# juanmc2005/diart

Hardware: NVIDIA H100
Metric: audio-seconds/sec (real-time factor) at 5s/0.5s step, batch 256 (higher is better)
Workload: dtype f32

## Files before the change

### diart_b200/_lib.py

```python
from __future__ import annotations

import ctypes as C
import os
from typing import Dict, Optional

import numpy as np
import torch

_HERE = os.path.dirname(os.path.abspath(__file__))
LIB_PATH = os.path.join(_HERE, "libdiartb200.so")

_lib: Optional[C.CDLL] = None


class DgTensor(C.Structure):
    _fields_ = [("name", C.c_char_p), ("data", C.c_void_p), ("numel", C.c_int64)]


_P = C.c_void_p
SIGNATURES = {
    "dg_last_error": (C.c_char_p, []),
    "dg_version": (C.c_int, []),
    "dg_launch_count": (C.c_int64, []),
    "dg_profile_enable": (C.c_int, [C.c_int]),
    "dg_profile_report": (C.c_int, [C.c_char_p, C.c_int]),
    "dg_selftest_gemm_tc": (C.c_int, [C.c_int, C.c_int, C.c_int, C.c_int, C.c_int, C.c_int, C.POINTER(C.c_float),
                                      C.POINTER(C.c_float)]),
    "dg_selftest_gemm_tc_grid": (C.c_int, [C.c_int, C.c_int, C.c_int, C.c_int, C.c_int, C.c_int, C.POINTER(C.c_int)]),
    "dg_selftest_gemm_tc_bounds": (C.c_int, [C.c_int, C.c_int, C.c_int, C.c_int, C.POINTER(C.c_int), C.POINTER(C.c_int),
                                             C.POINTER(C.c_int)]),
    "dg_selftest_wgmma_row_shift": (C.c_int, [C.c_int, C.POINTER(C.c_uint)]),
    "dg_selftest_wgmma_b_row_shift": (C.c_int, [C.c_int, C.POINTER(C.c_uint)]),
    "dg_selftest_gemm_tc_pool3_simt": (C.c_int, [C.c_int, C.c_int, C.c_int, C.c_int, C.c_int, C.POINTER(C.c_float),
                                                 C.POINTER(C.c_float), C.POINTER(C.c_int)]),
    "dg_selftest_gemm_tc_halo": (C.c_int, [C.c_int, C.c_int, C.c_int, C.c_int, C.c_int, C.c_int, C.POINTER(C.c_int),
                                           C.POINTER(C.c_int)]),
    "dg_selftest_split_f16_host": (C.c_int, [_P, C.c_longlong, _P, _P]),
    "dg_seg_create": (C.c_int, [C.POINTER(DgTensor), C.c_int, C.c_int, C.POINTER(_P)]),
    "dg_seg_dims": (C.c_int, [_P, C.c_int, C.POINTER(C.c_int), C.POINTER(C.c_int)]),
    "dg_seg_set_powerset": (C.c_int, [_P, C.c_int, C.c_int]),
    "dg_seg_forward": (C.c_int, [_P, _P, C.c_int, C.c_int, _P, _P]),
    "dg_seg_destroy": (C.c_int, [_P]),
    "dg_emb_create": (C.c_int, [C.POINTER(DgTensor), C.c_int, C.c_int, C.c_int, C.POINTER(_P)]),
    "dg_emb_dims": (C.c_int, [_P, C.c_int, C.POINTER(C.c_int), C.POINTER(C.c_int)]),
    "dg_emb_forward": (C.c_int, [_P, _P, _P, C.c_int, C.c_int, C.c_int, C.c_int, C.c_int, C.c_float, _P, _P]),
    "dg_emb_forward_rows": (C.c_int, [_P, _P, _P, C.c_int, C.c_int, C.c_int, _P, _P]),
    "dg_emb_destroy": (C.c_int, [_P]),
    "dg_emb_debug_trunk": (C.c_int, [_P, _P, C.c_int, C.c_int, C.c_int, _P, C.c_int64, _P]),
    "dg_seg_debug_stage": (C.c_int, [_P, _P, C.c_int, C.c_int, C.c_int, C.c_int, _P, C.c_int64, _P]),
    "dg_emb_debug_stage": (C.c_int, [_P, _P, _P, C.c_int, C.c_int, C.c_int, C.c_int, C.c_int, C.c_int, _P, C.c_int64, _P]),
    "dg_selftest_sinc_filters_host": (C.c_int, [_P, _P, _P]),
    "dg_selftest_fbank_tables_host": (C.c_int, [_P, _P]),
    "dg_osp": (C.c_int, [_P, C.c_int, C.c_int, C.c_int, C.c_float, C.c_float, C.c_int, _P, _P]),
    "dg_normalize_embeddings": (C.c_int, [_P, C.c_int, C.c_int, C.c_float, _P, _P]),
    "dg_cluster_create": (C.c_int, [C.c_int, C.c_int, C.c_double, C.c_double, C.c_double, C.c_int, C.POINTER(_P)]),
    "dg_cluster_set_metric": (C.c_int, [_P, C.c_int]),
    "dg_cluster_step": (C.c_int, [_P, _P, _P, C.c_int, C.c_int, C.c_int, _P, _P, _P]),
    "dg_cluster_reset": (C.c_int, [_P]),
    "dg_cluster_get_state": (C.c_int, [_P, _P, _P, C.POINTER(C.c_int)]),
    "dg_cluster_set_state": (C.c_int, [_P, _P, _P, C.c_int]),
    "dg_cluster_destroy": (C.c_int, [_P]),
    "dg_cluster_record_len": (C.c_int, [_P]),
    "dg_cluster_export_delta": (C.c_int, [_P, _P, _P]),
    "dg_cluster_merge": (C.c_int, [_P, _P, C.c_int, C.c_int, _P, C.c_int, _P]),
    "dg_pipeline_identity_export": (C.c_int, [_P, _P, _P]),
    "dg_pipeline_identity_merge": (C.c_int, [_P, _P, C.c_int, C.c_int, _P]),
    "dg_pipeline_create": (C.c_int, [_P, _P, _P, C.c_float, C.c_float, C.c_int, C.POINTER(_P)]),
    "dg_pipeline_set_hop": (C.c_int, [_P, C.c_int]),
    "dg_pipeline_step": (C.c_int, [_P, _P, C.c_int, C.c_int, _P, _P, _P, _P, _P]),
    "dg_pipeline_step_host": (C.c_int, [_P, _P, C.c_int, C.c_int, _P, _P, _P, _P]),
    "dg_pipeline_submit": (C.c_int, [_P, _P, C.c_int, C.c_int, _P]),
    "dg_pipeline_collect": (C.c_int, [_P, C.POINTER(_P), C.POINTER(_P), C.POINTER(_P), _P]),
    "dg_pipeline_collect_copy": (C.c_int, [_P, _P, _P, _P, _P]),
    "dg_pipeline_submit_host": (C.c_int, [_P, _P, C.c_int, C.c_int]),
    "dg_pipeline_collect_host": (C.c_int, [_P, _P, _P, _P]),
    "dg_pipeline_destroy": (C.c_int, [_P]),
    "dg_pipeline_nets_sets": (C.c_int, [_P, _P, C.c_int, C.c_int, C.c_int, _P, _P, _P, _P, C.c_int64, _P]),
    "dg_post_create": (C.c_int, [C.c_int, C.c_int, C.c_int, C.c_int, _P, C.c_double, C.c_int, C.POINTER(_P)]),
    "dg_post_step": (C.c_int, [_P, _P, _P, C.c_int, _P, _P, _P, C.c_int, C.POINTER(C.c_int), _P]),
    "dg_post_reset": (C.c_int, [_P]),
    "dg_post_destroy": (C.c_int, [_P]),
    "dg_stream_create": (C.c_int, [C.c_int, C.c_int, C.c_int, C.c_int, C.POINTER(_P)]),
    "dg_stream_push_host": (C.c_int, [_P, _P, C.c_int]),
    "dg_stream_available": (C.c_int, [_P]),
    "dg_stream_windows": (C.c_int, [_P, C.c_int, _P, _P]),
    "dg_stream_reset": (C.c_int, [_P]),
    "dg_stream_destroy": (C.c_int, [_P]),
    "dg_pipeline_submit_stream": (C.c_int, [_P, _P, C.c_int]),
    "dg_pipeline_call_stream": (C.c_int, [_P, _P, _P, C.c_int, _P, _P, _P, C.c_int, C.POINTER(C.c_int), _P, _P]),
    "dg_pipeline_call_host": (C.c_int, [_P, _P, _P, C.c_int, C.c_int, _P, _P, _P, C.c_int, C.POINTER(C.c_int), _P, _P]),
    "dg_pipeline_last_call_h2d_bytes": (C.c_int64, [_P]),
    "dg_resample_create": (C.c_int, [C.c_int, C.c_int, _P, C.c_int, C.c_int, C.POINTER(_P)]),
    "dg_resample_out_len": (C.c_int64, [_P, C.c_int64]),
    "dg_resample_forward": (C.c_int, [_P, _P, C.c_int, C.c_int64, _P, _P]),
    "dg_resample_destroy": (C.c_int, [_P]),
    "dg_stream_create_resampled": (C.c_int, [C.c_int, C.c_int, _P, C.c_int, C.c_int, C.POINTER(_P)]),
    "dg_stream_crop_host": (C.c_int, [_P, C.c_int, _P, _P]),
    "dg_sweep_create": (C.c_int, [C.c_int, C.c_int, C.c_int, C.c_int, C.c_int, _P, C.c_int, C.POINTER(_P)]),
    "dg_sweep_run": (C.c_int, [_P, _P, _P, C.c_int, _P, C.c_int, _P, _P, _P, _P, _P, C.c_int, C.POINTER(C.c_int), _P]),
    "dg_sweep_destroy": (C.c_int, [_P]),
    "dg_sweep_set_scored_regions": (C.c_int, [_P, C.c_int, _P, _P]),
    "dg_sweep_set_trial_sets": (C.c_int, [_P, C.c_int, _P, C.c_int]),
    "dg_sweep_set_seeds": (C.c_int, [_P, C.c_int, _P, _P]),
    "dg_sweep_set_identities": (C.c_int, [_P, C.c_int, _P]),
    "dg_sweep_score": (C.c_int, [_P, _P, _P, C.c_int, _P, C.c_int, _P, _P, _P, C.c_double, C.c_double, _P, _P, C.c_int,
                                 C.c_int, _P, _P, _P, C.c_int, _P]),
    "dg_sweep_run_files": (C.c_int, [_P, _P, _P, C.c_int, C.c_int, _P, _P, C.c_int, _P, _P, _P, _P, _P, C.c_int,
                                     C.POINTER(C.c_int), _P]),
    "dg_sweep_score_files": (C.c_int, [_P, _P, _P, C.c_int, C.c_int, _P, _P, C.c_int, _P, _P, _P, _P, C.c_double, _P, _P,
                                       _P, _P, _P, _P, _P, C.c_int, _P]),
    "dg_sweep_state_order": (C.c_int, [C.c_int, _P, C.c_int, _P]),
    "dg_sweep_run_latencies": (C.c_int, [_P, _P, _P, C.c_int, C.c_int, _P, C.c_int, C.c_int, _P, _P, _P, C.c_int, _P, _P,
                                         _P, _P, C.c_int, C.POINTER(C.c_int), _P]),
    "dg_sweep_score_latencies": (C.c_int, [_P, _P, _P, C.c_int, C.c_int, _P, C.c_int, C.c_int, _P, _P, _P, C.c_int, _P, _P,
                                           _P, _P, C.c_double, _P, _P, _P, _P, _P, _P]),
    "dg_sweep_check_latencies": (C.c_int, [C.c_int, C.c_int, _P, C.c_int, C.c_int, _P, _P, _P, C.c_int, C.c_int]),
    "dg_vad_sweep_curve_latencies": (C.c_int, [_P, _P, C.c_int, C.c_int, _P, C.c_int, C.c_int, _P, _P, _P, _P]),
    "dg_vad_sweep_create": (C.c_int, [C.c_int, C.c_int, C.c_int, _P, C.c_int, C.POINTER(_P)]),
    "dg_vad_sweep_curve": (C.c_int, [_P, _P, C.c_int, C.c_int, _P, _P, _P]),
    "dg_vad_sweep_run_files": (C.c_int, [_P, _P, C.c_int, _P, _P, C.c_int, C.POINTER(C.c_int), _P]),
    "dg_vad_sweep_score_files": (C.c_int, [_P, _P, C.c_int, _P, _P, _P, C.c_double, _P, _P, _P, _P]),
    "dg_vad_sweep_destroy": (C.c_int, [_P]),
    "dg_vad_sweep_set_scored_regions": (C.c_int, [_P, C.c_int, _P, _P]),
    "dg_multi_create": (C.c_int, [_P, _P, C.c_int, C.c_int, C.c_int, C.c_int, C.c_int, C.c_double, C.c_double, C.c_double,
                                  C.c_float, C.c_float, C.c_int, C.c_int, _P, C.POINTER(_P)]),
    "dg_multi_create_vad": (C.c_int, [_P, C.c_int, C.c_int, C.c_int, C.c_int, C.c_double, C.c_int, _P, C.POINTER(_P)]),
    "dg_multi_open": (C.c_int, [_P, C.c_int]),
    "dg_multi_close": (C.c_int, [_P, C.c_int]),
    "dg_multi_push_host": (C.c_int, [_P, C.c_int, _P, C.c_int]),
    "dg_multi_available": (C.c_int, [_P, C.c_int]),
    "dg_multi_step": (C.c_int, [_P, _P, C.c_int, _P, _P, _P, C.c_int, C.POINTER(C.c_int), _P, _P, _P]),
    "dg_multi_last_step_ms": (C.c_int, [_P, C.POINTER(C.c_float)]),
    "dg_multi_destroy": (C.c_int, [_P]),
    "dg_selftest_multi_staging_host": (C.c_int, [C.c_int, C.c_int, C.c_int, _P, _P, _P, _P]),
    "dg_multi_add_rate": (C.c_int, [_P, _P, C.c_int, C.c_int, C.POINTER(C.c_int)]),
    "dg_multi_open_rate": (C.c_int, [_P, C.c_int, C.c_int]),
    "dg_multi_open_config": (C.c_int, [_P, C.c_int, C.c_int, C.c_int, _P]),
    "dg_multi_open_seeded": (C.c_int, [_P, C.c_int, C.c_int, C.c_int, _P, _P, C.c_int]),
    "dg_multi_get_state": (C.c_int, [_P, C.c_int, _P, _P, C.POINTER(C.c_int)]),
    "dg_multi_last_windows": (C.c_int, [_P, _P, C.c_int]),
    "dg_gallery_create": (C.c_int, [_P, C.c_int, C.c_int, C.c_int, C.POINTER(_P)]),
    "dg_gallery_destroy": (C.c_int, [_P]),
    "dg_gallery_query": (C.c_int, [_P, _P, C.c_int, _P, _P, C.c_double, _P, _P, _P]),
    "dg_multi_set_gallery": (C.c_int, [_P, _P, C.c_double]),
    "dg_multi_set_names": (C.c_int, [_P, C.c_int, C.c_uint32, _P]),
    "dg_multi_set_slot_gallery": (C.c_int, [_P, C.c_int, _P, C.c_double]),
    "dg_selftest_gallery_plan_host": (C.c_int, [C.c_int, _P, C.c_int, _P, _P, _P, _P, _P, C.c_int, _P]),
    "dg_selftest_multi_gallery_host": (C.c_int, [C.c_int, C.c_int, C.c_int, C.c_int, _P, C.c_int, _P, _P, C.c_char_p,
                                                 C.c_int]),
    "dg_multi_last_names": (C.c_int, [_P, _P, C.c_int, C.POINTER(C.c_int)]),
    "dg_selftest_multi_frames_host": (C.c_int, [C.c_int, C.c_int, C.c_int, C.c_int, C.c_int, _P, C.c_int, _P, _P, _P, C.c_int,
                                                C.POINTER(C.c_int)]),
    "dg_multi_export_bytes": (C.c_int, [_P, _P, C.c_int, _P]),
    "dg_multi_export": (C.c_int, [_P, _P, C.c_int, C.c_int, _P, C.c_int64]),
    "dg_multi_import": (C.c_int, [_P, _P, C.c_int64, C.c_int, _P, _P]),
    "dg_selftest_multi_transfer_host": (C.c_int, [_P, C.c_int, _P, _P, _P, C.c_int, C.c_int, _P, _P, _P, C.c_int64, _P,
                                                  C.c_char_p, C.c_int]),
}


class DiartB200Error(RuntimeError):
    pass


def lib() -> C.CDLL:
    global _lib
    if _lib is not None:
        return _lib
    from . import build as _build

    if not os.path.exists(LIB_PATH) or (_build._stale() and _build.have_nvcc()):
        _build.build()
    try:
        handle = C.CDLL(LIB_PATH)
    except OSError as e:
        raise DiartB200Error(f"cannot load {LIB_PATH}: {e}. Run `python -m diart_b200.build`.") from e
    for name, (res, args) in SIGNATURES.items():
        fn = getattr(handle, name)
        fn.restype, fn.argtypes = res, args
    _lib = handle
    return handle


def check(rc: int):
    if rc == 0:
        return
    msg = lib().dg_last_error().decode()
    if rc == -1:
        if "Cannot update unknown centers" in msg:
            raise AssertionError(msg)
        raise ValueError(msg)
    if rc == -3:
        raise KeyError(msg)
    raise DiartB200Error(f"libdiartb200 error {rc}: {msg}")


def require_cuda(device: torch.device):
    if device.type != "cuda":
        raise DiartB200Error(
            f"diart_b200 runs on CUDA devices only (got '{device}'); there is no CPU implementation")
    if not torch.cuda.is_available():
        raise DiartB200Error("diart_b200 needs a CUDA device (sm_90a); none is available")


def pack_state_dict(state: Dict[str, "torch.Tensor | np.ndarray"]):
    keep, items = [], []
    for name, value in state.items():
        arr = value.detach().cpu().numpy() if isinstance(value, torch.Tensor) else np.asarray(value)
        if arr.dtype.kind != "f":
            continue
        arr = np.ascontiguousarray(arr, dtype=np.float32)
        bname = name.encode()
        keep.extend([arr, bname])
        items.append(DgTensor(bname, arr.ctypes.data, arr.size))
    array = (DgTensor * len(items))(*items)
    keep.append(array)
    return array, len(items), keep


def stream_ptr(device: torch.device) -> int:
    return torch.cuda.current_stream(device).cuda_stream


def ptr(t: Optional[torch.Tensor]) -> Optional[int]:
    return None if t is None else t.data_ptr()
```

### diart_b200/csrc/api.cu

```cuda
#include <math.h>
#include <stdlib.h>
#include <string.h>

#include <map>
#include <sstream>
#include <vector>

#include "host.cuh"

namespace dg {

static thread_local std::string g_err;
std::atomic<long long> g_launches{0};
thread_local int g_sm_limit = 0;
void set_error(const std::string& msg) { g_err = msg; }

struct ProfRec {
  std::string name;
  cudaEvent_t a, b;
};
static bool g_prof = false;
static std::vector<ProfRec> g_recs;
static const bool g_trace = getenv("DG_TRACE_LAUNCHES") && getenv("DG_TRACE_LAUNCHES")[0] == '1';
ProfScope::ProfScope(const char* name_, cudaStream_t st_) : on(g_prof), st(st_), a(nullptr), b(nullptr), name(name_) {
  if (g_trace) first = g_launches.load();
  if (!on) return;
  cudaEventCreate(&a);
  cudaEventCreate(&b);
  cudaEventRecord(a, st);
}
ProfScope::~ProfScope() {
  if (g_trace) fprintf(stderr, "dg-trace %s %lld %lld\n", name, first, (long long)g_launches.load());
  if (!on) return;
  cudaEventRecord(b, st);
  g_recs.push_back({name, a, b});
}

int upload_u16(DevBuf& b, const std::vector<uint16_t>& h) {
  if (b.ensure(h.size() * 2)) return -2;
  DG_CUDA(cudaMemcpy(b.p, h.data(), h.size() * 2, cudaMemcpyHostToDevice));
  return 0;
}

int upload_split(WeightPlanes& w, const std::vector<float>& w_nk, int N, int Npad, int K) {
  std::vector<uint16_t> h((size_t)Npad * K), l((size_t)Npad * K);
  w.scale = weight_plane_scale(w_nk.data(), (size_t)N * K);
  w.Npad = Npad;
  w.K = K;
  split_weights_host(w_nk.data(), N, Npad, K, h.data(), l.data(), w.scale);
  return (upload_u16(w.hi, h) || upload_u16(w.lo, l)) ? DG_ECUDA : 0;
}

int set_weights(TcGemm& t, const WeightPlanes& w) {
  if (t.KW * t.Cin != w.K) {
    set_error(std::string(t.tag ? t.tag : "gemm_tc") + ": the launch reads K = " + std::to_string(t.KW * t.Cin) +
              " but the weight planes have K = " + std::to_string(w.K));
    return DG_EINVAL;
  }
  t.W_hi = w.hi.p;
  t.W_lo = w.lo.p;
  t.w_scale = w.scale;
  t.Npad = w.Npad;
  return 0;
}

int upload(DevBuf& b, const std::vector<float>& h) {
  if (b.ensure(h.size() * sizeof(float))) return -2;
  DG_CUDA(cudaMemcpy(b.p, h.data(), h.size() * sizeof(float), cudaMemcpyHostToDevice));
  return 0;
}

}

extern "C" const char* dg_last_error(void) { return g_err.c_str(); }
extern "C" int dg_version(void) { return 100; }
extern "C" int64_t dg_launch_count(void) { return (int64_t)g_launches.load(); }

extern "C" int dg_profile_enable(int enable) {
  g_prof = enable != 0;
  return DG_OK;
}

extern "C" int dg_profile_report(char* buf, int cap) {
  cudaDeviceSynchronize();
  std::map<std::string, std::pair<int, double>> agg;
  for (auto& r : g_recs) {
    float ms = 0.f;
    cudaEventElapsedTime(&ms, r.a, r.b);
    auto& e = agg[r.name];
    e.first++;
    e.second += ms;
    cudaEventDestroy(r.a);
    cudaEventDestroy(r.b);
  }
  g_recs.clear();
  std::ostringstream os;
  os << "{";
  bool first = true;
  for (auto& kv : agg) {
    if (!first) os << ", ";
    first = false;
    os << "\"" << kv.first << "\": {\"count\": " << kv.second.first << ", \"ms\": " << kv.second.second << "}";
  }
  os << "}";
  const std::string s = os.str();
  if (!buf || cap <= (int)s.size()) {
    set_error("dg_profile_report: buffer too small");
    return DG_EINVAL;
  }
  memcpy(buf, s.c_str(), s.size() + 1);
  return (int)s.size();
}

extern "C" int dg_selftest_split_f16_host(const float* x, long long n, unsigned short* hi, unsigned short* lo) {
  if (!x || !hi || !lo || n < 0) {
    set_error("dg_selftest_split_f16_host: null argument");
    return DG_EINVAL;
  }
  for (long long i = 0; i < n; i++) {
    hi[i] = host_f32_to_h16(x[i]);
    lo[i] = host_f32_to_h16(x[i] - host_h16_to_f32(hi[i]));
  }
  return DG_OK;
}

extern "C" int dg_selftest_gemm_tc(int M, int Cin, int KW, int dil, int N, int epi, float* max_abs_diff,
                                   float* out_rms) {
  if (M < 1 || Cin < 16 || Cin % 16 || KW < 1 || N % 4 || !max_abs_diff || !out_rms) {
    set_error("dg_selftest_gemm_tc: bad arguments");
    return DG_EINVAL;
  }
  const int K = KW * Cin, npad = N == 64 ? 64 : (N + 255) / 256 * 256;
  const long long Mtot = M;
  std::vector<float> A((size_t)Mtot * Cin), Wkn((size_t)K * N), Wnk((size_t)N * K), bias(N), bsc(N), bsh(N);
  uint32_t seed = 12345u;
  auto rnd = [&]() {
    seed = seed * 1664525u + 1013904223u;
    return ((seed >> 8) & 0xFFFF) / 65536.f - 0.5f;
  };
  static const float amp = getenv("DG_SELFTEST_AMP") ? (float)atof(getenv("DG_SELFTEST_AMP")) : 2.f;
  for (auto& v : A) v = amp * rnd();
  for (int k = 0; k < K; k++)
    for (int n = 0; n < N; n++) {
      const float w = rnd() * 0.25f;
      Wkn[(size_t)k * N + n] = w;
      Wnk[(size_t)n * K + k] = w;
    }
  for (int n = 0; n < N; n++) {
    bias[n] = rnd();
    bsc[n] = 1.f + rnd();
    bsh[n] = rnd();
  }
  DevBuf dA, dWkn, dB, dS, dH, dAh, dAl, dC0, dC1, dOh, dOl;
  WeightPlanes dW;
  if (upload(dA, A) || upload(dWkn, Wkn) || upload(dB, bias) || upload(dS, bsc) || upload(dH, bsh) ||
      upload_split(dW, Wnk, N, npad, K))
    return DG_ECUDA;
  if (dAh.ensure((size_t)Mtot * Cin * 2) || dAl.ensure((size_t)Mtot * Cin * 2) || dC0.ensure((size_t)M * N * 4) ||
      dC1.ensure((size_t)M * N * 4) || dOh.ensure((size_t)M * N * 2) || dOl.ensure((size_t)M * N * 2))
    return DG_ECUDA;
  int rc;
  GemmArgs g{};
  g.A = dA.as<float>(); g.lda = Cin; g.Cin = Cin; g.KW = KW; g.dil = dil; g.Mtot = Mtot; g.M = M;
  g.W = dWkn.as<float>(); g.ldw = N; g.N = N; g.bias = dB.as<float>(); g.bn_scale = dS.as<float>();
  g.bn_shift = dH.as<float>(); g.C = dC0.as<float>(); g.ldc = N; g.epi = epi == 0 ? EPI_BIAS : EPI_BIAS_LEAKY_BN;
  g.tag = "selftest_simt";
  if ((rc = launch_gemm(g, nullptr))) return rc;
  if ((rc = launch_split_ex(dA.as<float>(), Mtot, Cin, Cin, Cin, 0, 1, nullptr, nullptr, dAh.p, dAl.p, nullptr))) return rc;
  TcGemm t{};
  t.A_hi = dAh.p; t.A_lo = dAl.p; t.lda = Cin; t.Cin = Cin; t.KW = KW; t.dil = dil; t.Mtot = Mtot; t.M = M;
  t.N = N; t.bias = dB.as<float>(); t.bn_scale = dS.as<float>();
  t.bn_shift = dH.as<float>(); t.out_f32 = dC1.as<float>(); t.out_hi = dOh.p; t.out_lo = dOl.p; t.ldc = N;
  t.epi = epi; t.tag = "selftest_tc";
  if ((rc = set_weights(t, dW)) || (rc = launch_gemm_tc(t, nullptr))) return rc;
  DG_CUDA(cudaDeviceSynchronize());
  std::vector<float> c0((size_t)M * N), c1((size_t)M * N);
  DG_CUDA(cudaMemcpy(c0.data(), dC0.p, c0.size() * 4, cudaMemcpyDeviceToHost));
  std::vector<uint16_t> oh, ol;
  if (epi == 1) {
    oh.resize((size_t)M * N);
    ol.resize((size_t)M * N);
    DG_CUDA(cudaMemcpy(oh.data(), dOh.p, oh.size() * 2, cudaMemcpyDeviceToHost));
    DG_CUDA(cudaMemcpy(ol.data(), dOl.p, ol.size() * 2, cudaMemcpyDeviceToHost));
    for (size_t i = 0; i < c1.size(); i++) c1[i] = host_h16_to_f32(oh[i]) + host_h16_to_f32(ol[i]);
  } else {
    DG_CUDA(cudaMemcpy(c1.data(), dC1.p, c1.size() * 4, cudaMemcpyDeviceToHost));
  }
  double md = 0, ss = 0;
  size_t worst = 0, n_big = 0;
  for (size_t i = 0; i < c0.size(); i++) {
    const double d = fabs((double)c0[i] - (double)c1[i]);
    if (!(d <= md)) {
      md = d;
      worst = i;
    }
    if (!(d <= 1e-2)) n_big++;
    ss += (double)c0[i] * c0[i];
  }
  if (n_big)
    fprintf(stderr, "dg_selftest_gemm_tc: %zu of %zu outputs differ by more than 1e-2; worst at row %zu col %zu: simt %g, wgmma %g\n",
            n_big, c0.size(), worst / N, worst % N, c0[worst], c1[worst]);
  if (n_big && epi == 1) {
    size_t shown = 0;
    for (size_t i = 0; i < c0.size() && shown < 12; i++)
      if (!(fabs((double)c0[i] - (double)c1[i]) <= 1e-2)) {
        fprintf(stderr, "   row %zu col %zu: simt %g, planes hi 0x%04x lo 0x%04x\n", i / N, i % N, c0[i], oh[i], ol[i]);
        shown++;
      }
  }
  *max_abs_diff = (float)md;
  *out_rms = (float)sqrt(ss / c0.size());
  return DG_OK;
}

extern "C" int dg_selftest_gemm_tc_grid(int M, int Cin, int KW, int dil, int N, int epi, int* equal) {
  if (M < 1 || Cin % 64 || KW < 1 || KW > 9 || N < 1 || N % 4 || epi < 0 || epi > 5 || !equal ||
      (epi == 3 && (KW != 9 || dil < 3 || M % (dil * dil) || N % 32)) || (epi == 5 && (N > 64 || M % 888))) {
    set_error("dg_selftest_gemm_tc_grid: bad arguments");
    return DG_EINVAL;
  }
  const int K = KW * Cin;
  const int npad = epi == 5 || N == 64 ? 64 : (epi == 3 && N == 32 ? 32 : (N + 127) / 128 * 128);
  const int ldc = epi == 3 ? (N + 31) / 32 * 32 : N;
  const int item_rows = epi == 4 ? 296 : 888, tile_rows = epi == 5 ? gemm_tc_pool3_tile_rows(item_rows) : 128;
  const long long m_tiles = (M + tile_rows - 1) / tile_rows;
  uint32_t seed = 777u;
  auto rnd = [&]() {
    seed = seed * 1664525u + 1013904223u;
    return ((seed >> 8) & 0xFFFF) / 65536.f - 0.5f;
  };
  std::vector<float> A((size_t)M * Cin), Wnk((size_t)N * K), bias(N), bsc(N), bsh(N), res((size_t)M * ldc), pw((size_t)M * 4);
  for (auto& v : A) v = 2.f * rnd();
  for (auto& v : Wnk) v = 0.25f * rnd();
  for (int n = 0; n < N; n++) {
    bias[n] = rnd();
    bsc[n] = 1.f + rnd();
    bsh[n] = rnd();
  }
  for (auto& v : res) v = rnd();
  for (auto& v : pw) v = rnd() + 0.5f;
  const size_t f32_bytes = epi == 0 || epi == 2 ? (size_t)M * ldc * 4 : (epi == 5 ? (size_t)(M / 3) * ldc * 4 : 0);
  const size_t plane_bytes = epi == 1 || epi == 3 ? (size_t)M * ldc * 2 : 0;
  const size_t part_bytes = epi == 4 ? (size_t)m_tiles * 2 * TC_POOL_SLOTS * N * 4 : (epi == 5 ? (size_t)m_tiles * 2 * TC_POOL3_SLOTS * N * 4 : 0);
  DevBuf dA, dAh, dAl, dB, dS, dH, dRes, dRh, dRl, dPw, dF, dOh, dOl, dPart;
  WeightPlanes dW;
  if (upload(dA, A) || upload(dB, bias) || upload(dS, bsc) || upload(dH, bsh) || upload(dRes, res) || upload(dPw, pw) ||
      upload_split(dW, Wnk, N, npad, K))
    return DG_ECUDA;
  if (dAh.ensure((size_t)M * Cin * 2) || dAl.ensure((size_t)M * Cin * 2) || dRh.ensure((size_t)M * ldc * 2) ||
      dRl.ensure((size_t)M * ldc * 2) || dF.ensure(f32_bytes + 4) || dOh.ensure(plane_bytes + 4) ||
      dOl.ensure(plane_bytes + 4) || dPart.ensure(part_bytes + 4))
    return DG_ECUDA;
  int rc;
  if ((rc = launch_split_ex(dA.as<float>(), M, Cin, Cin, Cin, 0, 1, nullptr, nullptr, dAh.p, dAl.p, nullptr)) ||
      (rc = launch_split_ex(dRes.as<float>(), M, ldc, ldc, ldc, 0, 1, nullptr, nullptr, dRh.p, dRl.p, nullptr)))
    return rc;
  int taps[9];
  for (int j = 0; j < 9; j++) taps[j] = (j / 3 - 1) * dil + (j % 3 - 1);
  TcGemm t{};
  t.A_hi = dAh.p; t.A_lo = dAl.p; t.lda = Cin; t.Cin = Cin; t.KW = KW; t.dil = dil; t.Mtot = M; t.M = M;
  t.N = N; t.bias = dB.as<float>(); t.bn_scale = dS.as<float>(); t.bn_shift = dH.as<float>(); t.ldc = ldc;
  t.epi = epi; t.tag = "selftest_tc_grid";
  t.out_f32 = f32_bytes ? dF.as<float>() : nullptr;
  t.out_hi = plane_bytes ? dOh.p : nullptr;
  t.out_lo = plane_bytes ? dOl.p : nullptr;
  if (epi == 3) {
    t.tap_off = taps; t.Wp = t.Wop = t.Hp = t.Hop = dil; t.relu = 1;
    t.res_hi = dRh.p; t.res_lo = dRl.p;
  }
  if (epi == 4) {
    t.pool_w = dPw.as<float>(); t.pool_part = dPart.as<float>(); t.pool_item_rows = item_rows; t.pool_K = 3; t.pool_T = item_rows;
  }
  if (epi == 5) {
    t.pool_part = dPart.as<float>(); t.pool_item_rows = item_rows; t.pool3_T = item_rows / 3 - 2;
    t.pool3_tile_rows = tile_rows;
  }
  if ((rc = set_weights(t, dW))) return rc;
  std::vector<unsigned char> first, cur;
  *equal = 1;
  const int caps[4] = {0, 1, 3, 7};
  for (int ci = 0; ci < 4; ci++) {
    DG_CUDA(cudaMemset(dF.p, 0, f32_bytes + 4));
    DG_CUDA(cudaMemset(dOh.p, 0, plane_bytes + 4));
    DG_CUDA(cudaMemset(dOl.p, 0, plane_bytes + 4));
    DG_CUDA(cudaMemset(dPart.p, 0, part_bytes + 4));
    {
      SmLimit cap(caps[ci]);
      if ((rc = launch_gemm_tc(t, nullptr))) return rc;
    }
    DG_CUDA(cudaDeviceSynchronize());
    cur.resize(f32_bytes + 2 * plane_bytes + part_bytes);
    DG_CUDA(cudaMemcpy(cur.data(), dF.p, f32_bytes, cudaMemcpyDeviceToHost));
    DG_CUDA(cudaMemcpy(cur.data() + f32_bytes, dOh.p, plane_bytes, cudaMemcpyDeviceToHost));
    DG_CUDA(cudaMemcpy(cur.data() + f32_bytes + plane_bytes, dOl.p, plane_bytes, cudaMemcpyDeviceToHost));
    DG_CUDA(cudaMemcpy(cur.data() + f32_bytes + 2 * plane_bytes, dPart.p, part_bytes, cudaMemcpyDeviceToHost));
    if (ci == 0)
      first.swap(cur);
    else if (cur != first)
      *equal = 0;
  }
  return DG_OK;
}

extern "C" int dg_selftest_wgmma_row_shift(int base_offset_mode, unsigned* ok_shifts) {
  if (base_offset_mode < 0 || base_offset_mode > 1 || !ok_shifts) {
    set_error("dg_selftest_wgmma_row_shift: bad arguments");
    return DG_EINVAL;
  }
  return selftest_wgmma_row_shift(base_offset_mode, ok_shifts) ? DG_ECUDA : DG_OK;
}

extern "C" int dg_selftest_wgmma_b_row_shift(int base_offset_mode, unsigned* ok_shifts) {
  if (base_offset_mode < 0 || base_offset_mode > 1 || !ok_shifts) {
    set_error("dg_selftest_wgmma_b_row_shift: bad arguments");
    return DG_EINVAL;
  }
  return selftest_wgmma_b_row_shift(base_offset_mode, ok_shifts) ? DG_ECUDA : DG_OK;
}

extern "C" int dg_selftest_gemm_tc_pool3_simt(int M, int Cin, int KW, int dil, int N, float* max_abs_diff, float* out_rms,
                                              int* ws) {
  if (M < 888 || M % 888 || Cin < 16 || Cin % 16 || Cin > 128 || KW < 2 || KW > 9 || dil < 1 || N < 1 || N > 64 || N % 4 ||
      !max_abs_diff || !out_rms || !ws) {
    set_error("dg_selftest_gemm_tc_pool3_simt: bad arguments");
    return DG_EINVAL;
  }
  const int K = KW * Cin, item_rows = 888, tile_rows = gemm_tc_pool3_tile_rows(item_rows);
  const long long m_tiles = (M + tile_rows - 1) / tile_rows, tail = (long long)(KW - 1) * dil;
  uint32_t seed = 4242u;
  auto rnd = [&]() {
    seed = seed * 1664525u + 1013904223u;
    return ((seed >> 8) & 0xFFFF) / 65536.f - 0.5f;
  };
  std::vector<float> A((size_t)(M + tail) * Cin, 0.f), Wkn((size_t)K * N), Wnk((size_t)N * K), bias(N);
  for (size_t i = 0; i < (size_t)M * Cin; i++) A[i] = 2.f * rnd();
  for (int k = 0; k < K; k++)
    for (int n = 0; n < N; n++) Wkn[(size_t)k * N + n] = Wnk[(size_t)n * K + k] = 0.25f * rnd();
  for (auto& v : bias) v = rnd();
  DevBuf dA, dWkn, dB, dAh, dAl, dC0, dP, dPart;
  WeightPlanes dW;
  if (upload(dA, A) || upload(dWkn, Wkn) || upload(dB, bias) || upload_split(dW, Wnk, N, 64, K)) return DG_ECUDA;
  if (dAh.ensure((size_t)M * Cin * 2) || dAl.ensure((size_t)M * Cin * 2) || dC0.ensure((size_t)M * N * 4) ||
      dP.ensure((size_t)(M / 3) * N * 4) || dPart.ensure((size_t)m_tiles * 2 * TC_POOL3_SLOTS * N * 4))
    return DG_ECUDA;
  int rc;
  GemmArgs g{};
  g.A = dA.as<float>(); g.lda = Cin; g.Cin = Cin; g.KW = KW; g.dil = dil; g.Mtot = M + tail; g.M = M;
  g.W = dWkn.as<float>(); g.ldw = N; g.N = N; g.bias = dB.as<float>(); g.C = dC0.as<float>(); g.ldc = N; g.epi = EPI_BIAS;
  g.tag = "selftest_simt";
  if ((rc = launch_gemm(g, nullptr))) return rc;
  if ((rc = launch_split_ex(dA.as<float>(), M, Cin, Cin, Cin, 0, 1, nullptr, nullptr, dAh.p, dAl.p, nullptr))) return rc;
  TcGemm t{};
  t.A_hi = dAh.p; t.A_lo = dAl.p; t.lda = Cin; t.Cin = Cin; t.KW = KW; t.dil = dil; t.Mtot = M; t.M = M;
  t.N = N; t.bias = dB.as<float>(); t.out_f32 = dP.as<float>(); t.ldc = N; t.epi = 5; t.tag = "selftest_tc_pool3";
  t.pool_part = dPart.as<float>(); t.pool_item_rows = item_rows; t.pool3_T = item_rows / 3 - 2; t.pool3_tile_rows = tile_rows;
  if ((rc = set_weights(t, dW))) return rc;
  *ws = gemm_tc_ws(t) ? 1 : 0;
  if ((rc = launch_gemm_tc(t, nullptr))) return rc;
  DG_CUDA(cudaDeviceSynchronize());
  std::vector<float> c0((size_t)M * N), p1((size_t)(M / 3) * N);
  DG_CUDA(cudaMemcpy(c0.data(), dC0.p, c0.size() * 4, cudaMemcpyDeviceToHost));
  DG_CUDA(cudaMemcpy(p1.data(), dP.p, p1.size() * 4, cudaMemcpyDeviceToHost));
  double md = 0, ss = 0;
  for (long long r = 0; r < M / 3; r++)
    for (int n = 0; n < N; n++) {
      const float* x = &c0[(size_t)(3 * r) * N + n];
      const double ref = std::max(std::max(x[0], x[N]), x[2 * N]);
      const double d = fabs(ref - (double)p1[(size_t)r * N + n]);
      if (!(d <= md)) md = d;
      ss += ref * ref;
    }
  *max_abs_diff = (float)md;
  *out_rms = (float)sqrt(ss / p1.size());
  return DG_OK;
}

extern "C" int dg_selftest_gemm_tc_halo(int M, int Cin, int KW, int dil, int N, int epi, int* equal, int* halo) {
  const bool folded = Cin % 64 != 0;
  if (M < 1 || Cin < 16 || Cin % 16 || Cin > 128 || KW < 2 || KW > 9 || dil < 1 || N < 1 || N % 4 ||
      (epi != 0 && epi != 1 && epi != 2 && epi != 5) || (epi == 1 && N % 32) || (epi == 5 && (N > 64 || M % 888)) ||
      (folded && dil != 1) || !equal || !halo) {
    set_error("dg_selftest_gemm_tc_halo: bad arguments");
    return DG_EINVAL;
  }
  const int K = KW * Cin, Kf = folded ? (K + 63) / 64 * 64 : K;
  const int npad = epi == 5 || N == 64 ? 64 : (N + 127) / 128 * 128;
  const int item_rows = 888, tile_rows = epi == 5 ? gemm_tc_pool3_tile_rows(item_rows) : 128;
  const long long m_tiles = (M + tile_rows - 1) / tile_rows;
  const long long tail = 64;
  uint32_t seed = 9090u;
  auto rnd = [&]() {
    seed = seed * 1664525u + 1013904223u;
    return ((seed >> 8) & 0xFFFF) / 65536.f - 0.5f;
  };
  std::vector<float> A((size_t)(M + tail) * Cin, 0.f), Wnk((size_t)N * K), Wf((size_t)N * Kf, 0.f), bias(N), bsc(N), bsh(N);
  for (size_t i = 0; i < (size_t)M * Cin; i++) A[i] = 2.f * rnd();
  for (auto& v : Wnk) v = 0.25f * rnd();
  for (int n = 0; n < N; n++)
    for (int k = 0; k < K; k++) Wf[(size_t)n * Kf + k] = Wnk[(size_t)n * K + k];
  for (int n = 0; n < N; n++) {
    bias[n] = rnd();
    bsc[n] = 1.f + rnd();
    bsh[n] = rnd();
  }
  const size_t f32_bytes = epi == 0 || epi == 2 ? (size_t)M * N * 4 : (epi == 5 ? (size_t)(M / 3) * N * 4 : 0);
  const size_t plane_bytes = epi == 1 ? (size_t)M * N * 2 : 0;
  const size_t part_bytes = epi == 5 ? (size_t)m_tiles * 2 * TC_POOL3_SLOTS * N * 4 : 0;
  DevBuf dA, dAh, dAl, dB, dS, dH, dF, dOh, dOl, dPart;
  WeightPlanes dW, dWf;
  if (upload(dA, A) || upload(dB, bias) || upload(dS, bsc) || upload(dH, bsh) || upload_split(dW, Wnk, N, npad, K) ||
      upload_split(dWf, Wf, N, npad, Kf))
    return DG_ECUDA;
  if (dAh.ensure((size_t)(M + tail) * Cin * 2) || dAl.ensure((size_t)(M + tail) * Cin * 2) || dF.ensure(f32_bytes + 4) ||
      dOh.ensure(plane_bytes + 4) || dOl.ensure(plane_bytes + 4) || dPart.ensure(part_bytes + 4))
    return DG_ECUDA;
  int rc;
  if ((rc = launch_split_ex(dA.as<float>(), M + tail, Cin, Cin, Cin, 0, 1, nullptr, nullptr, dAh.p, dAl.p, nullptr))) return rc;
  TcGemm t{};
  t.A_hi = dAh.p; t.A_lo = dAl.p; t.lda = Cin; t.Cin = Cin; t.KW = KW; t.dil = dil; t.Mtot = M; t.M = M;
  t.N = N; t.bias = dB.as<float>(); t.bn_scale = dS.as<float>(); t.bn_shift = dH.as<float>(); t.ldc = N;
  t.epi = epi; t.tag = "selftest_tc_halo";
  t.out_f32 = f32_bytes ? dF.as<float>() : nullptr;
  t.out_hi = plane_bytes ? dOh.p : nullptr;
  t.out_lo = plane_bytes ? dOl.p : nullptr;
  if (epi == 5) {
    t.pool_part = dPart.as<float>(); t.pool_item_rows = item_rows; t.pool3_T = item_rows / 3 - 2;
    t.pool3_tile_rows = tile_rows;
  }
  if ((rc = set_weights(t, dW))) return rc;
  *halo = gemm_tc_halo(t) ? 1 : 0;
  TcGemm ref = t;
  ref.tap_boxes = 1;
  if (folded) {
    ref.Cin = Kf;
    ref.KW = 1;
    if ((rc = set_weights(ref, dWf))) return rc;
  }
  std::vector<unsigned char> first, cur;
  *equal = 1;
  for (int run = 0; run < 3; run++) {
    DG_CUDA(cudaMemset(dF.p, 0, f32_bytes + 4));
    DG_CUDA(cudaMemset(dOh.p, 0, plane_bytes + 4));
    DG_CUDA(cudaMemset(dOl.p, 0, plane_bytes + 4));
    DG_CUDA(cudaMemset(dPart.p, 0, part_bytes + 4));
    {
      SmLimit cap(run == 1 ? 3 : 0);
      if ((rc = launch_gemm_tc(run == 2 ? ref : t, nullptr))) return rc;
    }
    DG_CUDA(cudaDeviceSynchronize());
    cur.resize(f32_bytes + 2 * plane_bytes + part_bytes);
    DG_CUDA(cudaMemcpy(cur.data(), dF.p, f32_bytes, cudaMemcpyDeviceToHost));
    DG_CUDA(cudaMemcpy(cur.data() + f32_bytes, dOh.p, plane_bytes, cudaMemcpyDeviceToHost));
    DG_CUDA(cudaMemcpy(cur.data() + f32_bytes + plane_bytes, dOl.p, plane_bytes, cudaMemcpyDeviceToHost));
    DG_CUDA(cudaMemcpy(cur.data() + f32_bytes + 2 * plane_bytes, dPart.p, part_bytes, cudaMemcpyDeviceToHost));
    if (run == 0)
      first.swap(cur);
    else if (cur != first)
      *equal = 0;
  }
  return DG_OK;
}

extern "C" int dg_selftest_gemm_tc_bounds(int M, int Cin, int N, int epi, int* outside_unchanged, int* equal, int* refused) {
  const bool planes = epi == 1;
  if (M < 1 || Cin < 64 || Cin % 64 || N < 1 || N % (planes ? 32 : 4) || epi < 0 || epi > 2 || !outside_unchanged || !equal ||
      !refused) {
    set_error("dg_selftest_gemm_tc_bounds: bad arguments");
    return DG_EINVAL;
  }
  const int npad = N <= 64 && epi == 0 ? 64 : (N + 127) / 128 * 128, esize = planes ? 2 : 4;
  const int ldc = N + 40;
  const long long rows = (long long)M + 130;
  uint32_t seed = 4242u;
  auto rnd = [&]() {
    seed = seed * 1664525u + 1013904223u;
    return ((seed >> 8) & 0xFFFF) / 65536.f - 0.5f;
  };
  std::vector<float> A((size_t)M * Cin), Wnk((size_t)N * Cin), bias(N), bsc(N), bsh(N);
  for (auto& v : A) v = 2.f * rnd();
  for (auto& v : Wnk) v = 0.25f * rnd();
  for (int n = 0; n < N; n++) {
    bias[n] = rnd();
    bsc[n] = 1.f + rnd();
    bsh[n] = rnd();
  }
  const size_t dense_bytes = (size_t)M * N * esize, wide_bytes = (size_t)rows * ldc * esize + 16;
  DevBuf dA, dAh, dAl, dB, dS, dH, dD0, dD1, dW0, dW1;
  WeightPlanes dW;
  if (upload(dA, A) || upload(dB, bias) || upload(dS, bsc) || upload(dH, bsh) || upload_split(dW, Wnk, N, npad, Cin) ||
      dAh.ensure((size_t)M * Cin * 2) || dAl.ensure((size_t)M * Cin * 2) || dD0.ensure(dense_bytes) ||
      dD1.ensure(dense_bytes) || dW0.ensure(wide_bytes) || dW1.ensure(wide_bytes))
    return DG_ECUDA;
  int rc;
  if ((rc = launch_split_ex(dA.as<float>(), M, Cin, Cin, Cin, 0, 1, nullptr, nullptr, dAh.p, dAl.p, nullptr))) return rc;
  TcGemm t{};
  t.A_hi = dAh.p; t.A_lo = dAl.p; t.lda = Cin; t.Cin = Cin; t.KW = 1; t.dil = 1; t.Mtot = M; t.M = M;
  t.N = N; t.bias = dB.as<float>(); t.bn_scale = dS.as<float>(); t.bn_shift = dH.as<float>();
  t.epi = epi; t.tag = "selftest_tc_bounds";
  if ((rc = set_weights(t, dW))) return rc;
  auto point = [&](DevBuf& o0, DevBuf& o1, size_t off, int ld) {
    unsigned char* b0 = static_cast<unsigned char*>(o0.p) + off;
    unsigned char* b1 = static_cast<unsigned char*>(o1.p) + off;
    t.out_f32 = planes ? nullptr : reinterpret_cast<float*>(b0);
    t.out_hi = planes ? b0 : nullptr;
    t.out_lo = planes ? b1 : nullptr;
    t.ldc = ld;
  };
  const unsigned char SENTINEL = 0xA5;
  DG_CUDA(cudaMemset(dW0.p, SENTINEL, wide_bytes));
  DG_CUDA(cudaMemset(dW1.p, SENTINEL, wide_bytes));
  point(dD0, dD1, 0, N);
  if ((rc = launch_gemm_tc(t, nullptr))) return rc;
  point(dW0, dW1, 0, ldc);
  if ((rc = launch_gemm_tc(t, nullptr))) return rc;
  point(dW0, dW1, (size_t)esize, ldc);
  const int rc_base = launch_gemm_tc(t, nullptr);
  point(dW0, dW1, 0, ldc + (planes ? 4 : 2));
  const int rc_pitch = launch_gemm_tc(t, nullptr);
  DG_CUDA(cudaDeviceSynchronize());
  const int n_out = planes ? 2 : 1;
  std::vector<unsigned char> dense(dense_bytes), wide(wide_bytes);
  *outside_unchanged = 1;
  *equal = 1;
  for (int o = 0; o < n_out; o++) {
    DG_CUDA(cudaMemcpy(dense.data(), (o ? dD1 : dD0).p, dense_bytes, cudaMemcpyDeviceToHost));
    DG_CUDA(cudaMemcpy(wide.data(), (o ? dW1 : dW0).p, wide_bytes, cudaMemcpyDeviceToHost));
    const size_t row_bytes = (size_t)N * esize, pitch = (size_t)ldc * esize;
    for (long long r = 0; r < rows; r++) {
      const unsigned char* w = wide.data() + r * pitch;
      const bool inside = r < M;
      if (inside && memcmp(w, dense.data() + r * row_bytes, row_bytes)) *equal = 0;
      for (size_t b = inside ? row_bytes : 0; b < pitch; b++)
        if (w[b] != SENTINEL) *outside_unchanged = 0;
    }
    for (size_t b = (size_t)rows * pitch; b < wide_bytes; b++)
      if (wide[b] != SENTINEL) *outside_unchanged = 0;
  }
  *refused = rc_base == DG_EINVAL && rc_pitch == DG_EINVAL;
  return DG_OK;
}
```

### diart_b200/csrc/dg_common.cuh

```cuda
#pragma once
#include <cuda_runtime.h>
#include <stdint.h>
#include <stdio.h>

#include <atomic>
#include <string>
#include <vector>

namespace dg {

void set_error(const std::string& msg);
extern std::atomic<long long> g_launches;
extern thread_local int g_sm_limit;
inline int usable_sms() {
  int dev = 0, sms = 132;
  cudaGetDevice(&dev);
  cudaDeviceGetAttribute(&sms, cudaDevAttrMultiProcessorCount, dev);
  return (g_sm_limit > 0 && g_sm_limit < sms) ? g_sm_limit : sms;
}

#define DG_CUDA(expr)                                                                   \
  do {                                                                                  \
    cudaError_t _e = (expr);                                                            \
    if (_e != cudaSuccess) {                                                            \
      dg::set_error(std::string(#expr) + ": " + cudaGetErrorString(_e));                \
      return -2;                                                                        \
    }                                                                                   \
  } while (0)

inline bool first_use_on_device(bool* flags) {
  int dev = 0;
  cudaGetDevice(&dev);
  if (dev < 0 || dev >= 64) return true;
  if (flags[dev]) return false;
  flags[dev] = true;
  return true;
}

#define DG_LAUNCHED()                                                                   \
  do {                                                                                  \
    dg::g_launches.fetch_add(1, std::memory_order_relaxed);                             \
    cudaError_t _e = cudaGetLastError();                                                \
    if (_e != cudaSuccess) {                                                            \
      dg::set_error(std::string("kernel launch failed at ") + __FILE__ + ":" +          \
                    std::to_string(__LINE__) + ": " + cudaGetErrorString(_e));          \
      return -2;                                                                        \
    }                                                                                   \
  } while (0)

struct ProfScope {
  bool on;
  cudaStream_t st;
  cudaEvent_t a, b;
  const char* name;
  long long first = 0;
  ProfScope(const char* name, cudaStream_t st);
  ~ProfScope();
};

struct Geom {
  int S;
  int T0c;
  int T0;
  int T1;
  int T2;
  int S0, S1, S2;
};
inline Geom make_geom(int S) {
  Geom g;
  g.S = S;
  g.T0c = (S - 251) / 10 + 1;
  g.T0 = g.T0c / 3;
  g.T1 = (g.T0 - 4) / 3;
  g.T2 = (g.T1 - 4) / 3;
  g.S2 = g.T2 + 3;
  while ((g.S2 * 9) < g.T0 + 0 || (g.S2 * 3) < g.T1) g.S2++;
  g.S1 = g.S2 * 3;
  g.S0 = g.S1 * 3;
  return g;
}

__device__ __forceinline__ float leaky(float x) { return x > 0.f ? x : 0.01f * x; }

int launch_wave_stats(const float* wav, int B, int S, float* mean, float* rstd, cudaStream_t st, const int* skip_flag = nullptr);
bool stream_stats_ok(int S, int hop);
size_t stream_stats_doubles(int B, int S, int hop);
int launch_stream_stats(const float* wav, int B, int S, int hop, double* part, float* mean, float* rstd, const int* flag,
                        cudaStream_t st);
int launch_instnorm_stats(const float* x, int B, int stride_rows, int T, int C, int ldc, const float* gamma,
                          const float* beta, float* sc, float* sh, cudaStream_t st, int pool = 0, const int* skip_flag = nullptr);
int launch_instnorm_finalize(const float* part, int B, int item_rows, int tile_rows, int T, int C, int N, const float* bias,
                             const float* gamma, const float* beta, float* sc, float* sh, int ld, cudaStream_t st);
enum Epi { EPI_BIAS = 0, EPI_BIAS_LEAKY_BN = 2 };
struct GemmArgs {
  const float* A;
  int lda;
  int Cin;
  int KW, dil;
  long long Mtot;
  long long M;
  const float* W;
  int ldw;
  int N;
  const float* bias;
  const float* bn_scale;
  const float* bn_shift;
  float* C;
  int ldc;
  int epi;
  const char* tag;
};
int launch_gemm(const GemmArgs& a, cudaStream_t st);
constexpr int TC_POOL_SLOTS = 9, TC_POOL3_SLOTS = 3;
struct TcGemm {
  const void* A_hi;
  const void* A_lo;
  int lda, Cin, KW, dil;
  long long Mtot, M;
  const void* W_hi;
  const void* W_lo;
  float w_scale;
  int Npad, N;
  const float* bias;
  const float* bn_scale;
  const float* bn_shift;
  float* out_f32;
  void* out_hi;
  void* out_lo;
  int ldc;
  int epi;
  const char* tag;
  const int* tap_off;
  int Wp, Hp, Wop, Hop, stride2, relu;
  const void* res_hi;
  const void* res_lo;
  const float* pool_w;
  float* pool_part;
  int pool_item_rows, pool_K;
  int pool_T;
  int pool3_T, pool3_tile_rows;
  int tap_boxes;
};
inline int gemm_tc_pool3_tile_rows(int item_rows) {
  for (int t = 126; t >= 96; t -= 3)
    if (item_rows % t == 0) return t;
  return 0;
}
int launch_gemm_tc(const TcGemm& g, cudaStream_t st);
bool gemm_tc_halo(const TcGemm& g);
bool gemm_tc_ws(const TcGemm& g);
int selftest_wgmma_row_shift(int base_offset_mode, unsigned* ok_shifts);
int selftest_wgmma_b_row_shift(int base_offset_mode, unsigned* ok_shifts);
int launch_split_ex(const float* x, long long rows_out, int C, int ld_in, int ld_out, int pool, int item_rows,
                    const float* sc, const float* sh, void* hi, void* lo, cudaStream_t st, const int* skip_flag = nullptr);
void split_weights_host(const float* w, int N, int Npad, int K, uint16_t* hi, uint16_t* lo, float scale = 1.f);
float weight_plane_scale(const float* w, size_t n);
uint16_t host_f32_to_h16(float f);
float host_h16_to_f32(uint16_t h);
int sinc_tc_rows_per_item(const Geom& g);
size_t sinc_tc_plane_elems(int B, const Geom& g);
void sinc_tc_pack_filters(const float* filt, uint16_t* planes );
void sinc_tc_affine_consts(const float* filt, float beta, float* cf);
int launch_sinc_prep(const float* wav, const float* mean, const float* rstd, int B, const Geom& g, void* planes_hi,
                     void* planes_lo, cudaStream_t st, const int* skip_flag = nullptr);
int launch_sinc0_tc(float gamma, const float* cf_dev, const void* w_planes, int B, const Geom& g, const void* planes_hi,
                    const void* planes_lo, float* p0, cudaStream_t st, const int* skip_flag = nullptr);
struct SincStreamGeom {
  int Ls;
  int P;
  int rows;
  size_t plane;
};
SincStreamGeom sinc_stream_geom(int B, const Geom& g, int hop);
int launch_overlap_check(const float* wav, int B, int S, int hop, int* flag, cudaStream_t st);
int launch_stream_prep(const float* wav, const float* rstd, int B, const Geom& g, int hop, void* planes_hi, void* planes_lo,
                       int* flag, cudaStream_t st);
int launch_sinc0_tc_stream(const void* w_planes, int B, const Geom& g, int hop, const void* planes_hi, const void* planes_lo,
                           float* craw, const int* flag, cudaStream_t st);
size_t sinc_pool_part_floats(int B, const Geom& g, int hop);
int launch_sinc_pool_fused(const float* craw, const float* mean, const float* rstd, const float* cf, const float* hsum, float gamma,
                           int B, const Geom& g, int hop, const float* g0, const float* b0, float* part, float* sc, float* sh,
                           void* planes_hi, void* planes_lo, const int* flag, cudaStream_t st);
size_t lstm_tc_plane_elems();
int lstm_tc_rows(int B);
int lstm_tc_ctas(int B);
float lstm_tc_pack_whh(const float* whh_fwd, const float* whh_bwd, uint16_t* hi, uint16_t* lo);
int launch_lstm_layer_tc(const float* gx, const void* whh_hi, const void* whh_lo, float w_scale, int B, int T, int stride,
                         float* hout, void* out_hi, void* out_lo, cudaStream_t st);
int launch_seg_final(const float* y , const float* wc , const float* bc, int B, int T,
                     int stride, int K, float* seg , cudaStream_t st);
int launch_seg_powerset(const float* y, const float* wc, const float* bc, int B, int T, int stride, int C, int num_speakers,
                        const unsigned* masks_dev, float* seg , cudaStream_t st);
int launch_osp(const float* seg, int B, int F, int K, float gamma, float beta, int normalize, float* out,
               cudaStream_t st);
constexpr int DG_MAX_OSP_SETS = 64;
struct OspSets {
  float gamma[DG_MAX_OSP_SETS], beta[DG_MAX_OSP_SETS];
  int normalize[DG_MAX_OSP_SETS];
};
int launch_osp_sets(const float* seg, int B, int F, int K, const OspSets& sets, int G, float* out, cudaStream_t st);
int launch_stats_pool(const float* x , int B, int stride, int T, int C, const float* w ,
                      int F, int K, const int* idx0, const int* idx1, const float* lam1, float eps,
                      float* pooled , cudaStream_t st, long long item_pitch = 0, int row_pitch = 0);
int launch_pool_weights(const float* w , int B, int F, int K, int item_rows, int T, const int* idx0, const int* idx1,
                        const float* lam1, float eps, float* row_w , float* vsum , cudaStream_t st);
int launch_pool_weights_sets(const float* w, int B, int G, int F, int K, int item_rows, int T, const int* idx0, const int* idx1,
                             const float* lam1, float eps, float* row_w, long long rw_stride, float* vsum, cudaStream_t st);
int launch_pool_finalize(const float* part, const float* row_w, const float* vsum, const float* pivot, int B, int K, int C,
                         int item_rows, int T, float eps, float* pooled , cudaStream_t st);
int launch_l2norm(const float* in, int rows, int D, float norm, float* out, cudaStream_t st);
int launch_row_equal_flags(const float* wav, int N, int S, int* flags, cudaStream_t st);
int launch_gather_rows(const float* src, const int* index, int rows, int cols, float* dst, cudaStream_t st);
int launch_fb_planes(const float* wav, int B, int S, void* hi, void* lo, float* inv_scale, float* level, cudaStream_t st);
int launch_fb_mel(const float* spec, int ld, int rows_per_item, int T, int B, const float* inv_scale, const float* level,
                  const float* banks, const int* k_lo, const int* k_hi, float* logmel, cudaStream_t st);
int launch_fb_mean(const float* logmel, int B, int T, float* mean, cudaStream_t st);
int launch_rn_stem(const float* logmel, const float* mean, int B, int T, const float* w, const float* sc, const float* sh,
                   void* hi, void* lo, cudaStream_t st);
struct ClusterParams {
  int M, D;
  float tau_f, rho_f;
  double delta;
  int metric;
};
int launch_cluster_step(const ClusterParams& p, const float* seg, const float* emb, int B, int F, int K,
                        double* centers, int* active, int* initialized, float* prep ,
                        double* prep_d , int32_t* map, float* permuted, cudaStream_t st);
int launch_cluster_export(const double* centers, const int* active, const double* base, const int* base_active, int M,
                          int D, double* record, cudaStream_t st);
int launch_cluster_merge(const double* records, int world, int rank, const ClusterParams& p, int rec_len, double* centers,
                         int* active, double* base, int* base_active, int* initialized, int32_t* relabel,
                         cudaStream_t st);
int launch_relabel_maps(int32_t* maps, int n, const int32_t* relabel, cudaStream_t st);
int launch_cluster_sweep(const ClusterParams& p, const double* trials_dev, int T, const int2* states_dev, int S,
                         const int* chunk_off_dev, const float* seg, const float* emb, int B, int F, int K, double* centers,
                         int* active, int* initialized, float* prep, double* prep_d, int32_t* maps, cudaStream_t st,
                         bool own_rows = false);
int launch_cluster_sweep_sets(const ClusterParams& p, const double* trials_dev, int T, const int2* states_dev, int S,
                              const int* chunk_off_dev, const float* seg, const float* emb, int G, int B, int F, int K,
                              double* centers, int* active, int* initialized, float* prep, double* prep_d, int32_t* maps,
                              cudaStream_t st);
size_t cluster_prep_floats(int B, int K);
int launch_sweep_seed(const int* seed_off, const double* seeds, int nf, int T, int M, int D, double* centers, int* active,
                      int* initialized, cudaStream_t st);
int launch_post_virtual(const float* seg, const int32_t* map, int N, const int32_t* vchunk, int Nv, int F, int K, int M, int nw,
                        const int32_t* plan, int plan_stride, const double* hamming, const double* taus, int T,
                        int32_t* header, uint32_t* turns, int turn_cap, unsigned int* total, cudaStream_t st);
int launch_expand_windows(const float* ring, long long r0, int C, int hop, int S, int B, float* wav, cudaStream_t st);
struct RingPiece {
  long long src, dst;
  int slot, n;
};
struct TickSlot {
  int slot, row0, n, cur, n_hist, nw, pad[2];
};
int launch_ring_scatter(const float* staged, const RingPiece* pieces, int n_pieces, int C, float* rings, cudaStream_t st);
int launch_ring_gather(const float* rings, int C, const TickSlot* act, const int2* rows, const long long* start, int S, int B,
                       float* wav, cudaStream_t st);
int launch_post_slots(const float* seg, const int32_t* map, const float* hist_seg, const int32_t* hist_map,
                      const TickSlot* act, const int2* rows, int slots, int B, int F, int K, int M, int nw,
                      const int32_t* plan, int plan_stride, const double* hamming, const double* params, int32_t* header,
                      uint32_t* turns, int turn_cap, unsigned int* total, cudaStream_t st);
int launch_post_slots_history(const float* seg, const int32_t* map, float* hist_seg, int32_t* hist_map, const TickSlot* act,
                              int n_act, int slots, int F, int K, int nw, cudaStream_t st);
size_t cluster_prep_doubles(int B, int K);
int launch_der_hyp_count(const int32_t* header, const uint32_t* turns, int nf, const int* chunk_off, int T, int N, int M,
                         const double* out_start, const double* out_res, const double* shifts, double collar, int* offsets,
                         cudaStream_t st);
int launch_der_hyp_write(const int32_t* header, const uint32_t* turns, int nf, const int* chunk_off, int T, int N, int M,
                         const double* out_start, const double* out_res, const double* shifts, double collar, int* offsets,
                         double* segs, double* segs_copy, int copy_cap, cudaStream_t st);
constexpr int DER_ROFF = 33;
int launch_der_score(const int* hoff, const double* hseg, int nf, int T, int M, const int* roff, const int* R,
                     const double* rseg, double* comp, cudaStream_t st, const int* uoff = nullptr,
                     const double* useg = nullptr, const int* named = nullptr);
int launch_vad_curve_virtual(const float* seg, const int32_t* vchunk, int Nv, int F, int K, const int32_t* plan, int plan_stride,
                             const double* hamming, const long long* curve_off, double* curve, cudaStream_t st);
int launch_vad_binarize(const double* curve, const long long* curve_off, int N, int T, const double* taus, int32_t* header,
                        uint32_t* turns, int turn_cap, unsigned int* total, cudaStream_t st);
int launch_vad_slots(const float* seg, const float* hist_vad, const TickSlot* act, const int2* rows, int slots, int B, int F,
                     int K, int nw, const int32_t* plan, int plan_stride, const double* hamming, const double* params,
                     int32_t* header, uint32_t* turns, int turn_cap, unsigned int* total, cudaStream_t st);
int launch_vad_slots_history(const float* seg, float* hist_vad, const TickSlot* act, int n_act, int slots, int F, int K, int nw,
                             cudaStream_t st);
struct RsGeom {
  int o, n, w, T;
};
struct RsItem {
  long long start, len, j_lo, j_cnt, out_off;
};
struct RsJob {
  const float* x;
  long long C;
  const RsItem* items;
  RsItem base;
  long long start_step, out_step;
  const float* W;
  RsGeom g;
  float* out;
};
long long resample_out_len(const RsGeom& g, long long L);
bool resample_geom_ok(const RsGeom& g);
int launch_resample(const RsJob& j, int items, long long max_out, cudaStream_t st);
int launch_resample_stream(const float* ring, long long C, long long rpos, long long hop, long long L, int B, const float* W,
                           const RsGeom& g, float* ys, float* out, cudaStream_t st);
struct RsFrames {
  long long first;
  int slot, count;
};
struct RsRow {
  long long start, frame0;
  int slot, row;
};
int launch_resample_frames(const float* rings, long long C, const RsFrames* items, int n_items, long long max_count,
                           const float* W, const RsGeom& g, float* yrings, long long Y, long long Q, cudaStream_t st);
int launch_resample_gather(const float* rings, long long C, const float* yrings, long long Y, long long Q, const RsRow* rows,
                           int n_rows, long long r_lo, long long r_hi, const float* W, const RsGeom& g, long long L,
                           long long out_len, float* wav, cudaStream_t st);

void fbank_frame_operator(std::vector<float>& op );
void fbank_mel_banks(std::vector<float>& banks , std::vector<int>& k_lo, std::vector<int>& k_hi);

constexpr int GAL_TILE_E = 64, GAL_TILE_Q = 128, GAL_KC = 16, GAL_NAME_PREFIX = 1024;
struct GalGroup {
  const double* E;
  const double* En;
  double threshold;
  int G, tiles, per_split, splits, q_ub, seg0, seg1, pad;
};
struct GalWork {
  int group, tile, split;
};
int launch_gallery_norms(const double* E, int G, int Dp, double* En, cudaStream_t st);
int gallery_plan(std::vector<GalGroup>& groups, std::vector<GalWork>& work);
int launch_gallery_nearest(const GalGroup* groups, const GalWork* work, int n_work, const int2* gq, int Dp, const double* X,
                           int D, const int2* qd, int Qmax, const int32_t* claimed, double* part_d, int* part_e,
                           cudaStream_t st);
int launch_gallery_queries(const int2* segs, int n, const GalGroup* groups, int n_groups, const int* active,
                           const uint32_t* named, int M, int2* qd, int* seg_off, int2* gq, int* names, cudaStream_t st);
int launch_gallery_claim(const double* part_d, const int* part_e, int Qmax, const int2* qd, const int* seg_off,
                         const int2* segs, int n_seg, const GalGroup* groups, int32_t* claimed, int32_t* entry_out,
                         double* dist_out, uint32_t* named, int M, int* names, int32_t* list, int32_t* prefix, cudaStream_t st);

struct XferPiece {
  const uint32_t* src;
  uint32_t* dst;
  long long n, src_pos, src_mod, dst_pos, dst_mod;
};
int launch_slot_transfer(const XferPiece* pieces, int n_pieces, const char* tag, cudaStream_t st);

}
```

### diart_b200/csrc/gemm_tc.cu

```cuda
#include <cuda.h>
#include <cuda_bf16.h>
#include <math.h>
#include <stdlib.h>
#include <string.h>

#include <algorithm>
#include <map>
#include <mutex>
#include <string>
#include <utility>
#include <vector>

#include "dg_common.cuh"
#include "tc_ptx.cuh"

namespace dg {

constexpr int TC_BM = 128, TC_BK = 32, TC_THREADS = 384;
constexpr int TC_SMEM_MAX = 227 * 1024;

struct TcArgs {
  long long M;
  int N;
  int m_tiles, n_tiles;
  int KW, dil, cin_blocks;
  const float* bias;
  const float* bn_scale;
  const float* bn_shift;
  float* out_f32;
  __nv_bfloat16* out_hi;
  __nv_bfloat16* out_lo;
  int ldc;
  float acc_scale;
  int tap_off[9];
  int Wp, Hp, Wop, Hop, stride2, relu;
  const __nv_bfloat16* res_hi;
  const __nv_bfloat16* res_lo;
  const float* pool_w;
  float* pool_part;
  int pool_item_rows, pool_K, pool_T;
  int tile_rows, pool3_T;
  unsigned* tile_ctr;
  int halo_rows;
  int cin;
  int wblocks;
  int halo_bytes;
  int op_bytes;
};

enum TcEpi { TC_BIAS_F32 = 0, TC_LEAKY_BN_SPLIT = 1, TC_LEAKY_BN_F32 = 2, TC_CONV2D = 3, TC_POOL = 4, TC_MAXPOOL3 = 5 };

__host__ __device__ constexpr bool tc_pooling(int epi) { return epi == TC_POOL || epi == TC_MAXPOOL3; }
__host__ __device__ constexpr bool tc_box_store(int epi) { return epi == TC_BIAS_F32 || epi == TC_LEAKY_BN_SPLIT || epi == TC_LEAKY_BN_F32; }

template <int BN>
struct TcSmem {
  static constexpr int A_BYTES = TC_BM * TC_BK * 2;
  static constexpr int W_BYTES = BN * TC_BK * 2;
  static constexpr int STAGE_BYTES = 2 * A_BYTES + 2 * W_BYTES;
  static constexpr int W_STAGE_BYTES = 2 * W_BYTES;
  static constexpr int NSTAGE = BN == 128 ? 4 : 6;
  static constexpr int NSTAGE_HALO = BN == 128 ? 5 : 6;
  __host__ static int halo_bytes(int cin, int rows) { return (2 * ((cin + 31) / 32) * rows * 64 + 1023) / 1024 * 1024; }
  __host__ static int halo_op_bytes(int cin, int rows) { return 2 * halo_bytes(cin, rows) + NSTAGE_HALO * W_STAGE_BYTES; }
  static constexpr int BAR_BYTES = 256;
  static constexpr int PARAM_FLOATS = 3 * BN;
  static constexpr int CHUNK_W = 64;
  static constexpr int CHUNK_FLOATS = CHUNK_W / 32 * TC_BM * 33;
  __host__ __device__ static constexpr int extra_floats(int epi) { return epi == TC_POOL ? 128 * 4 + 4 * 2 * 8 * 32 : (epi == TC_MAXPOOL3 ? 4 * 2 * 2 * 32 : 0); }
  __host__ __device__ static constexpr int consumer_floats(int epi) { return PARAM_FLOATS + (tc_pooling(epi) ? CHUNK_FLOATS + extra_floats(epi) : 0); }
  static constexpr int ACC_LD = BN + 4;
  static constexpr int BOX_BYTES = TC_BM * 128;
  __host__ __device__ static constexpr int stage_tile_bytes(int epi) {
    return tc_pooling(epi) ? 0 : (epi == TC_CONV2D ? TC_BM * ACC_LD * 4 : TC_BM * BN * 4);
  }
  __host__ __device__ static constexpr int total(int epi, int op_bytes = NSTAGE * STAGE_BYTES) {
    return op_bytes + stage_tile_bytes(epi) + BAR_BYTES + 2 * consumer_floats(epi) * 4 + 1024;
  }
};
static_assert(TcSmem<128>::total(TC_POOL) <= TC_SMEM_MAX && TcSmem<64>::total(TC_MAXPOOL3) <= TC_SMEM_MAX &&
              TcSmem<128>::total(TC_CONV2D) <= TC_SMEM_MAX && TcSmem<64>::total(TC_CONV2D) <= TC_SMEM_MAX &&
              TcSmem<32>::total(TC_CONV2D) <= TC_SMEM_MAX && TcSmem<128>::total(TC_BIAS_F32) <= TC_SMEM_MAX,
              "gemm_tc: shared memory");

template <int BN, int EPI>
__device__ __forceinline__ void tc_stage_params(const TcArgs& a, float* params, int bar, int n0, int et) {
  named_sync(bar, 128);
  for (int i = et; i < BN; i += 128) {
    const int n = n0 + i;
    const bool ok = n < a.N;
    params[i] = (ok && a.bias) ? a.bias[n] : 0.f;
    constexpr bool has_bn = EPI != TC_BIAS_F32;
    params[BN + i] = (ok && has_bn) ? a.bn_scale[n] * (EPI == TC_CONV2D ? a.acc_scale : 1.f) : 1.f;
    params[2 * BN + i] = (ok && has_bn) ? a.bn_shift[n] : 0.f;
  }
  named_sync(bar, 128);
}

template <int BN, int EPI>
__device__ __forceinline__ void tc_box_epilogue(const TcArgs& a, const float* params, float (&acc)[2][BN / 2],
                                                uint32_t tile, int quad, int lane) {
  using S = TcSmem<BN>;
  const int r0 = 16 * quad + (lane >> 2), sw = lane >> 2, cq = lane & 3;
#pragma unroll
  for (int j = 0; j < BN / 8; j++) {
    const int col = 8 * j + 2 * cq;
    const float2 bias = *reinterpret_cast<const float2*>(params + col);
    float2 bsc = make_float2(1.f, 1.f), bsh = make_float2(0.f, 0.f);
    if (EPI != TC_BIAS_F32) {
      bsc = *reinterpret_cast<const float2*>(params + BN + col);
      bsh = *reinterpret_cast<const float2*>(params + 2 * BN + col);
    }
#pragma unroll
    for (int h = 0; h < 2; h++) {
#pragma unroll
      for (int e2 = 0; e2 < 2; e2++) {
        const int row = 64 * h + r0 + 8 * e2;
        float x0 = fmaf(acc[h][4 * j + 2 * e2], a.acc_scale, bias.x);
        float x1 = fmaf(acc[h][4 * j + 2 * e2 + 1], a.acc_scale, bias.y);
        if (EPI != TC_BIAS_F32) {
          x0 = fmaf(leaky(x0), bsc.x, bsh.x);
          x1 = fmaf(leaky(x1), bsc.y, bsh.y);
        }
        if (EPI == TC_LEAKY_BN_SPLIT) {
          uint16_t h0, l0, h1, l1;
          split_h16(x0, h0, l0);
          split_h16(x1, h1, l1);
          const int off = (j / 8) * S::BOX_BYTES + row * 128 + (((j & 7) ^ sw) << 4) + 4 * cq;
          st_shared_u32(tile + off, pack_u16x2(h0, h1));
          st_shared_u32(tile + (BN / 64) * S::BOX_BYTES + off, pack_u16x2(l0, l1));
        } else {
          const int q = 2 * (j & 3) + (cq >> 1);
          const int off = (j / 4) * S::BOX_BYTES + row * 128 + ((q ^ sw) << 4) + 8 * (cq & 1);
          st_shared_v2(tile + off, x0, x1);
        }
      }
    }
  }
}

__device__ __forceinline__ void acc_ld32(const float* p, uint32_t (&r)[32]) {
#pragma unroll
  for (int i = 0; i < 8; i++) {
    const float4 v = reinterpret_cast<const float4*>(p)[i];
    r[4 * i] = __float_as_uint(v.x);
    r[4 * i + 1] = __float_as_uint(v.y);
    r[4 * i + 2] = __float_as_uint(v.z);
    r[4 * i + 3] = __float_as_uint(v.w);
  }
}

template <int BN>
__device__ __forceinline__ void tc_conv2d_epilogue_tile(const TcArgs& a, const float* params, const float* acc_row,
                                                        long long mt, int n0, int quad, int lane) {
    const long long m = mt * TC_BM + quad * 32 + lane;
    long long mo = m;
    bool row_ok = m < a.M;
    {
      const unsigned mu = (unsigned)m, per = (unsigned)(a.Wp * a.Hp);
      const unsigned item = mu / per, rem = mu - item * per;
      const int w = (int)(rem / (unsigned)a.Hp), h = (int)(rem - (unsigned)w * (unsigned)a.Hp);
      row_ok = row_ok && w >= 1 && w <= a.Wp - 2 && h >= 1 && h <= a.Hp - 2;
      if (a.stride2) {
        row_ok = row_ok && (w & 1) && (h & 1);
        mo = ((long long)item * a.Wop + ((w - 1) >> 1) + 1) * a.Hop + ((h - 1) >> 1) + 1;
      }
    }
#pragma unroll 1
    for (int c = 0; c < BN; c += 32) {
      uint32_t r[32];
      acc_ld32(acc_row + c, r);
      if (n0 + c >= a.N) continue;
      float v[32];
#pragma unroll
      for (int i = 0; i < 32; i++) v[i] = fmaf(__uint_as_float(r[i]), params[BN + c + i], params[2 * BN + c + i]);
      if (row_ok && a.res_hi) {
        const uint4* rh = reinterpret_cast<const uint4*>(a.res_hi + mo * a.ldc + n0 + c);
        const uint4* rl = reinterpret_cast<const uint4*>(a.res_lo + mo * a.ldc + n0 + c);
#pragma unroll
        for (int q = 0; q < 4; q++) {
          const uint4 hq = rh[q], lq = rl[q];
          const uint32_t hw[4] = {hq.x, hq.y, hq.z, hq.w}, lw[4] = {lq.x, lq.y, lq.z, lq.w};
#pragma unroll
          for (int e = 0; e < 4; e++) {
            v[8 * q + 2 * e] += h16_to_f32((uint16_t)(hw[e] & 0xFFFFu)) + h16_to_f32((uint16_t)(lw[e] & 0xFFFFu));
            v[8 * q + 2 * e + 1] += h16_to_f32((uint16_t)(hw[e] >> 16)) + h16_to_f32((uint16_t)(lw[e] >> 16));
          }
        }
      }
      if (a.relu) {
#pragma unroll
        for (int i = 0; i < 32; i++) v[i] = fmaxf(v[i], 0.f);
      }
      if (row_ok) {
        if (a.out_f32) {
          float* po = a.out_f32 + mo * a.ldc + n0 + c;
#pragma unroll
          for (int i = 0; i < 8; i++)
            reinterpret_cast<float4*>(po)[i] = make_float4(v[4 * i], v[4 * i + 1], v[4 * i + 2], v[4 * i + 3]);
        }
        if (a.out_hi) {
          uint32_t hi[16], lo[16];
#pragma unroll
          for (int i = 0; i < 16; i++) {
            uint16_t h0, l0, h1, l1;
            split_h16(v[2 * i], h0, l0);
            split_h16(v[2 * i + 1], h1, l1);
            hi[i] = pack_u16x2(h0, h1);
            lo[i] = pack_u16x2(l0, l1);
          }
          uint4* ph = reinterpret_cast<uint4*>(a.out_hi + mo * a.ldc + n0 + c);
          uint4* pl = reinterpret_cast<uint4*>(a.out_lo + mo * a.ldc + n0 + c);
#pragma unroll
          for (int i = 0; i < 4; i++) {
            ph[i] = make_uint4(hi[4 * i], hi[4 * i + 1], hi[4 * i + 2], hi[4 * i + 3]);
            pl[i] = make_uint4(lo[4 * i], lo[4 * i + 1], lo[4 * i + 2], lo[4 * i + 3]);
          }
        }
      }
    }
}

template <bool STG_IN_DSM = false>
__device__ __forceinline__ void tc_maxpool3_cols(const TcArgs& a, const float* dsm, float* stg, const float* bias_c,
                                                 long long mt, int nc, int et, int bar) {
  {
    const int col = et & 31, rg = et >> 5, n = nc + col;
    const long long first = mt * (long long)a.tile_rows;
    const long long item0 = first / a.pool_item_rows;
    const long long nxt = (item0 + 1) * a.pool_item_rows;
    const int brow3 = nxt - first < a.tile_rows ? (int)(nxt - first) / 3 : a.tile_rows / 3;
    const long long p_first = first / 3;
    const int f0 = (int)(p_first - item0 * (a.pool_item_rows / 3));
    const long long Mp = a.M / 3;
    const float bias = bias_c[col];
    auto pooled = [&](int pr) {
      return fmaxf(fmaxf(dsm[(3 * pr) * 33 + col], dsm[(3 * pr + 1) * 33 + col]), dsm[(3 * pr + 2) * 33 + col]);
    };
    const float piv0 = pooled(0), piv1 = pooled(brow3 < a.tile_rows / 3 ? brow3 : 0);
    float s1[2] = {0.f, 0.f}, s2[2] = {0.f, 0.f};
    for (int pr = rg; pr < a.tile_rows / 3; pr += 4) {
      const float v = pooled(pr);
      const int sg = pr >= brow3 ? 1 : 0;
      const int frame = sg ? pr - brow3 : f0 + pr;
      const long long P = p_first + pr;
      if (P < Mp) {
        if (n < a.N) a.out_f32[P * a.ldc + n] = v + bias;
        if (frame < a.pool3_T) {
          const float dv = v - (sg ? piv1 : piv0);
          s1[sg] += dv;
          s2[sg] = fmaf(dv, dv, s2[sg]);
        }
      }
    }
    if (STG_IN_DSM) named_sync(bar, 128);
#pragma unroll
    for (int sg = 0; sg < 2; sg++) {
      stg[((rg * 2 + sg) * 2 + 0) * 32 + col] = s1[sg];
      stg[((rg * 2 + sg) * 2 + 1) * 32 + col] = s2[sg];
    }
    if (rg == 0 && n < a.N)
#pragma unroll
      for (int sg = 0; sg < 2; sg++) a.pool_part[(((size_t)mt * 2 + sg) * TC_POOL3_SLOTS + 2) * a.N + n] = sg ? piv1 : piv0;
  }
  named_sync(bar, 128);
  {
    const int col = et & 31, q = et >> 5, sg = q >> 1, j = q & 1, n = nc + col;
    const float tot = ((stg[((0 * 2 + sg) * 2 + j) * 32 + col] + stg[((1 * 2 + sg) * 2 + j) * 32 + col]) +
                       stg[((2 * 2 + sg) * 2 + j) * 32 + col]) + stg[((3 * 2 + sg) * 2 + j) * 32 + col];
    if (n < a.N) a.pool_part[(((size_t)mt * 2 + sg) * TC_POOL3_SLOTS + j) * a.N + n] = tot;
  }
  named_sync(bar, 128);
}

template <int BN, int EPI>
__device__ __forceinline__ void tc_pool_epilogue_tile(const TcArgs& a, float* params, float* chunk, float* pool_stage,
                                                 const float (&acc)[2][BN / 2], int bar, long long mt, int n0, int quad,
                                                 int lane, int et, bool stage_params) {
    const long long m = mt * (EPI == TC_MAXPOOL3 ? a.tile_rows : TC_BM) + quad * 32 + lane;
    if (stage_params) {
      named_sync(bar, 128);
      for (int i = et; i < BN; i += 128) {
        const int n = n0 + i;
        const bool ok = n < a.N;
        params[i] = (ok && a.bias) ? a.bias[n] : 0.f;
        constexpr bool has_bn = EPI != TC_BIAS_F32 && EPI != TC_MAXPOOL3;
        params[BN + i] = (ok && has_bn) ? a.bn_scale[n] : 1.f;
        params[2 * BN + i] = (ok && has_bn) ? a.bn_shift[n] : 0.f;
      }
      named_sync(bar, 128);
    }
    int brow = TC_BM, valid0 = 0, valid1 = 0;
    if (EPI == TC_POOL) {
      float4 pw = make_float4(0.f, 0.f, 0.f, 0.f);
      if (m < a.M) pw = *reinterpret_cast<const float4*>(a.pool_w + m * 4);
      reinterpret_cast<float4*>(pool_stage)[quad * 32 + lane] = pw;
      const long long first = (long long)mt * TC_BM;
      const long long nxt = (first / a.pool_item_rows + 1) * a.pool_item_rows;
      brow = nxt - first < TC_BM ? (int)(nxt - first) : TC_BM;
      valid0 = min(brow, max(0, a.pool_T - (a.pool_item_rows - (int)(nxt - first))));
      valid1 = max(0, min(TC_BM - brow, a.pool_T));
      named_sync(bar, 128);
    }
    constexpr int CW = TcSmem<BN>::CHUNK_W;
    const int fr0 = 16 * quad + (lane >> 2), fc0 = 2 * (lane & 3);
#pragma unroll
    for (int c0 = 0; c0 < BN; c0 += CW) {
      {
#pragma unroll
        for (int c = c0; c < c0 + CW; c += 32) {
          float* dsm = chunk + (c - c0) / 32 * (128 * 33);
#pragma unroll
          for (int jj = 0; jj < 4; jj++) {
#pragma unroll
            for (int e1 = 0; e1 < 2; e1++) {
              const int col = 8 * jj + fc0 + e1;
              float bb = 0.f, ss = 0.f, hh = 0.f;
              if (EPI == TC_POOL) bb = params[c + col], ss = params[BN + c + col], hh = params[2 * BN + c + col];
#pragma unroll
              for (int h = 0; h < 2; h++) {
#pragma unroll
                for (int e2 = 0; e2 < 2; e2++) {
                  const float y = acc[h][4 * (c / 8 + jj) + 2 * e2 + e1];
                  float* d = dsm + (64 * h + fr0 + 8 * e2) * 33 + col;
                  if (EPI == TC_POOL) {
                    const float x = leaky(fmaf(y, a.acc_scale, bb));
                    *d = fmaf(x, ss, hh) - hh;
                  } else {
                    *d = y * a.acc_scale;
                  }
                }
              }
            }
          }
        }
      }
      named_sync(bar, 128);
#pragma unroll
      for (int c = c0; c < c0 + CW; c += 32) {
        if (EPI == TC_POOL) {
          const float* dsm = chunk + (c - c0) / 32 * (128 * 33);
          const float4* wsm = reinterpret_cast<const float4*>(pool_stage);
          float* stg = pool_stage + 128 * 4;
          const int col = et & 31;
          auto pivot = [&](int lo, int n) {
            if (n <= 0) return 0.f;
            const float pa = dsm[lo * 33 + col], pb = dsm[(lo + n / 2) * 33 + col];
            return fabsf(pa + pb) > 16.f * fabsf(pa - pb) ? 0.5f * (pa + pb) : 0.f;
          };
          if (c != c0) named_sync(bar, 128);
          {
            const int rg = et >> 5, r_lo = rg * 32, r_hi = r_lo + 32;
#pragma unroll
            for (int sg = 0; sg < 2; sg++) {
              const int lo = sg == 0 ? r_lo : max(r_lo, brow), hi = sg == 0 ? min(r_hi, brow) : r_hi;
              const float piv = sg ? pivot(brow < TC_BM ? brow : 0, valid1) : pivot(0, valid0);
              float s1[4] = {0.f, 0.f, 0.f, 0.f}, s2[4] = {0.f, 0.f, 0.f, 0.f};
              if (a.pool_K <= 3) {
#pragma unroll 8
                for (int rr = lo; rr < hi; rr++) {
                  const float dv = dsm[rr * 33 + col] - piv;
                  const float4 w4 = wsm[rr];
                  const float a0 = w4.x * dv, a1 = w4.y * dv, a2 = w4.z * dv;
                  s1[0] += a0; s1[1] += a1; s1[2] += a2;
                  s2[0] = fmaf(a0, dv, s2[0]); s2[1] = fmaf(a1, dv, s2[1]); s2[2] = fmaf(a2, dv, s2[2]);
                }
              } else {
#pragma unroll 8
                for (int rr = lo; rr < hi; rr++) {
                  const float dv = dsm[rr * 33 + col] - piv;
                  const float4 w4 = wsm[rr];
                  const float a0 = w4.x * dv, a1 = w4.y * dv, a2 = w4.z * dv, a3 = w4.w * dv;
                  s1[0] += a0; s1[1] += a1; s1[2] += a2; s1[3] += a3;
                  s2[0] = fmaf(a0, dv, s2[0]); s2[1] = fmaf(a1, dv, s2[1]); s2[2] = fmaf(a2, dv, s2[2]); s2[3] = fmaf(a3, dv, s2[3]);
                }
              }
#pragma unroll
              for (int k = 0; k < 4; k++) {
                stg[((rg * 2 + sg) * 8 + 2 * k) * 32 + col] = s1[k];
                stg[((rg * 2 + sg) * 8 + 2 * k + 1) * 32 + col] = s2[k];
              }
            }
          }
          named_sync(bar, 128);
          {
            const int twoK = 2 * a.pool_K, n = n0 + c + col;
            for (int q = et >> 5; q < 2 * twoK; q += 4) {
              const int sg = q >= twoK ? 1 : 0, j = q - sg * twoK;
              const float tot = ((stg[((0 * 2 + sg) * 8 + j) * 32 + col] + stg[((1 * 2 + sg) * 8 + j) * 32 + col]) +
                                 stg[((2 * 2 + sg) * 8 + j) * 32 + col]) + stg[((3 * 2 + sg) * 8 + j) * 32 + col];
              if (n < a.N && mt < a.m_tiles) a.pool_part[(((size_t)mt * 2 + sg) * TC_POOL_SLOTS + j) * a.N + n] = tot;
            }
            if (et < 64 && n < a.N && mt < a.m_tiles) {
              const int sg = et >> 5;
              a.pool_part[(((size_t)mt * 2 + sg) * TC_POOL_SLOTS + 8) * a.N + n] = sg ? pivot(brow < TC_BM ? brow : 0, valid1)
                                                                                      : pivot(0, valid0);
            }
          }
          if (c + 32 == c0 + CW) named_sync(bar, 128);
          continue;
        }
        if (EPI == TC_MAXPOOL3) {
          tc_maxpool3_cols(a, chunk + (c - c0) / 32 * (128 * 33), pool_stage, params + c, mt, n0 + c, et, bar);
          continue;
        }
      }
    }
}

template <int BN, int EPI, bool HALO>
__global__ void __launch_bounds__(TC_THREADS, 1)
gemm_tc_kernel(const __grid_constant__ CUtensorMap tmA_hi, const __grid_constant__ CUtensorMap tmA_lo,
               const __grid_constant__ CUtensorMap tmW_hi, const __grid_constant__ CUtensorMap tmW_lo,
               const __grid_constant__ CUtensorMap tmC0, const __grid_constant__ CUtensorMap tmC1, TcArgs a) {
  using S = TcSmem<BN>;
  constexpr bool POOLING = tc_pooling(EPI);
  constexpr int NSTAGE = HALO ? S::NSTAGE_HALO : S::NSTAGE;
  extern __shared__ unsigned char smem_raw[];
  unsigned char* smem = reinterpret_cast<unsigned char*>((reinterpret_cast<uintptr_t>(smem_raw) + 1023) & ~uintptr_t(1023));
  unsigned char* ring = HALO ? smem + 2 * a.halo_bytes : smem;
  constexpr int RING_STAGE = HALO ? S::W_STAGE_BYTES : S::STAGE_BYTES;
  unsigned char* tile_s = smem + a.op_bytes;
  uint64_t* bars = reinterpret_cast<uint64_t*>(tile_s + S::stage_tile_bytes(EPI));
  uint64_t* full = bars;
  uint64_t* empty = bars + NSTAGE;
  uint64_t* tile_full = bars + 2 * NSTAGE;
  uint64_t* tile_empty = tile_full + 2;
  uint64_t* halo_full = tile_empty + 2;
  uint64_t* halo_empty = halo_full + 2;
  volatile int* tile_idx = reinterpret_cast<volatile int*>(halo_empty + 2);
  float* cons = reinterpret_cast<float*>(reinterpret_cast<unsigned char*>(bars) + S::BAR_BYTES);

  const int warp = __shfl_sync(0xffffffffu, (int)(threadIdx.x >> 5), 0), lane = threadIdx.x & 31;
  const int wg = warp >> 2;
  const int num_tiles = a.m_tiles * a.n_tiles;
  const int kblocks = HALO ? a.wblocks : a.KW * a.cin_blocks;
  const int halo_box = a.halo_rows * 64, halo_cb = (a.cin + 31) / 32;

  if (threadIdx.x == 0) {
    for (int s = 0; s < NSTAGE; s++) {
      mbar_init(&full[s], 1);
      mbar_init(&empty[s], 1);
    }
    for (int c = 0; c < 2; c++) {
      mbar_init(&tile_full[c], 1);
      mbar_init(&tile_empty[c], 128);
      mbar_init(&halo_full[c], 1);
      mbar_init(&halo_empty[c], 1);
    }
    asm volatile("fence.mbarrier_init.release.cluster;" ::: "memory");
  }
  __syncthreads();

  if (wg == 0) {
    setmaxnreg_dec<HALO ? 48 : 40>();
    if (threadIdx.x == 0) {
      int stage = 0, phase = 0, next = 0;
      bool halo_next = false;
      for (int i = 0, tile = blockIdx.x;; i++) {
        const int c = i & 1;
        mbar_wait(&tile_empty[c], ((i >> 1) & 1) ^ 1);
        if (tile >= num_tiles) {
          tile_idx[c] = -1;
          mbar_arrive(&tile_full[c]);
          mbar_wait(&tile_empty[c ^ 1], (((i + 1) >> 1) & 1) ^ 1);
          tile_idx[c ^ 1] = -2;
          mbar_arrive(&tile_full[c ^ 1]);
          break;
        }
        tile_idx[c] = tile;
        mbar_arrive(&tile_full[c]);
        const int mt = tile / a.n_tiles, nt = tile - mt * a.n_tiles;
        const int m0 = mt * (EPI == TC_MAXPOOL3 ? a.tile_rows : TC_BM), n0 = nt * BN;
        if constexpr (HALO) {
          auto load_halo = [&](int cc, int r0) {
            unsigned char* hs = smem + cc * a.halo_bytes;
            mbar_expect_tx(&halo_full[cc], 2 * halo_cb * halo_box);
            for (int cb = 0; cb < halo_cb; cb++) {
              tma_load_2d(hs + cb * halo_box, &tmA_hi, cb * TC_BK, r0, &halo_full[cc]);
              tma_load_2d(hs + (halo_cb + cb) * halo_box, &tmA_lo, cb * TC_BK, r0, &halo_full[cc]);
            }
          };
          if (!halo_next) {
            mbar_wait(&halo_empty[c], ((i >> 1) & 1) ^ 1);
            load_halo(c, m0);
          }
          halo_next = false;
          next = POOLING ? (int)gridDim.x + (int)atomicAdd(&a.tile_ctr[0], 1u) : tile + (int)gridDim.x;
          const int next_m0 = next / a.n_tiles * (EPI == TC_MAXPOOL3 ? a.tile_rows : TC_BM);
          const uint32_t next_par = (((i + 1) >> 1) & 1) ^ 1;
          for (int kb = 0; kb < kblocks; kb++) {
            const long long t0 = clock64();
            for (;;) {
              if (!halo_next && next < num_tiles && mbar_test_wait(&halo_empty[c ^ 1], next_par)) {
                load_halo(c ^ 1, next_m0);
                halo_next = true;
              }
              if (mbar_test_wait(&empty[stage], phase ^ 1)) break;
              if (clock64() - t0 > 4000000000LL) __trap();
            }
            unsigned char* st = ring + stage * RING_STAGE;
            mbar_expect_tx(&full[stage], S::W_STAGE_BYTES);
            tma_load_2d(st, &tmW_hi, kb * TC_BK, n0, &full[stage]);
            tma_load_2d(st + S::W_BYTES, &tmW_lo, kb * TC_BK, n0, &full[stage]);
            if (++stage == NSTAGE) {
              stage = 0;
              phase ^= 1;
            }
          }
        }
        for (int j = 0; j < (HALO ? 0 : a.KW); j++) {
          for (int cb = 0; cb < a.cin_blocks; cb++) {
            mbar_wait(&empty[stage], phase ^ 1);
            unsigned char* st = smem + stage * S::STAGE_BYTES;
            mbar_expect_tx(&full[stage], S::STAGE_BYTES);
            const int kcol = (j * a.cin_blocks + cb) * TC_BK;
            tma_load_2d(st, &tmA_hi, cb * TC_BK, m0 + a.tap_off[j], &full[stage]);
            tma_load_2d(st + S::A_BYTES, &tmA_lo, cb * TC_BK, m0 + a.tap_off[j], &full[stage]);
            tma_load_2d(st + 2 * S::A_BYTES, &tmW_hi, kcol, n0, &full[stage]);
            tma_load_2d(st + 2 * S::A_BYTES + S::W_BYTES, &tmW_lo, kcol, n0, &full[stage]);
            if (++stage == NSTAGE) {
              stage = 0;
              phase ^= 1;
            }
          }
        }
        if (!HALO) next = POOLING ? (int)gridDim.x + (int)atomicAdd(&a.tile_ctr[0], 1u) : tile + (int)gridDim.x;
        tile = next;
      }
      if (POOLING) {
        __threadfence();
        if (atomicAdd(&a.tile_ctr[1], 1u) == gridDim.x - 1) {
          atomicExch(&a.tile_ctr[0], 0u);
          atomicExch(&a.tile_ctr[1], 0u);
        }
      }
    }
    return;
  }
  setmaxnreg_inc<HALO ? 224 : 232>();
  const int c = wg - 1, quad = warp & 3, et = threadIdx.x - 128 * wg;
  float* params = cons + c * S::consumer_floats(EPI);
  float* chunk = params + S::PARAM_FLOATS;
  float* pool_stage = chunk + S::CHUNK_FLOATS;
  const int bar = 1 + c, turn = 3 + c, turn_other = 3 + (c ^ 1), acc_free = 5 + c, acc_free_other = 5 + (c ^ 1);
  if (c == 1) {
    named_arrive(3, 256);
    if (!POOLING) named_arrive(5, 256);
  }
  for (int n = 0;; n++) {
    mbar_wait(&tile_full[c], n & 1);
    const int tile = tile_idx[c];
    mbar_arrive(&tile_empty[c]);
    if (tc_box_store(EPI) && tile >= 0 && (a.n_tiles > 1 || n == 0))
      tc_stage_params<BN, EPI>(a, params, bar, (tile - tile / a.n_tiles * a.n_tiles) * BN, et);
    named_sync(turn, 256);
    if (tile < 0) {
      if (tile == -1) {
        named_arrive(turn_other, 256);
        if (!POOLING) named_sync(acc_free, 256);
      }
      break;
    }
    const int pos = (2 * n + c) * kblocks;
    int stage = pos % NSTAGE, phase = (pos / NSTAGE) & 1;
    float acc[2][BN / 2];
#pragma unroll
    for (int i = 0; i < BN / 2; i++) acc[0][i] = acc[1][i] = 0.f;
    uint32_t htap = 0;
    int hch = 0;
    if constexpr (HALO) mbar_wait(&halo_full[c], n & 1);
    const uint32_t hs = smem_u32(smem + c * a.halo_bytes);
    for (int kb = 0; kb < kblocks; kb++) {
      mbar_wait(&full[stage], phase);
      const uint32_t sa = smem_u32(ring + stage * RING_STAGE);
      const uint32_t sw = HALO ? sa : sa + 2 * S::A_BYTES;
      const uint64_t w_hi = wg_desc_sw64(sw), w_lo = wg_desc_sw64(sw + S::W_BYTES);
      constexpr uint64_t HALF = (uint64_t)((64 * TC_BK * 2) >> 4);
      wg_fence_acc(acc[0]);
      wg_fence_acc(acc[1]);
      wg_fence();
#pragma unroll
      for (int ks = 0; ks < TC_BK / 16; ks++) {
        const uint64_t adv = (uint64_t)((ks * 32) >> 4);
        uint64_t a_hi, a_lo;
        if constexpr (HALO) {
          const uint32_t aa = hs + (uint32_t)(hch >> 5) * halo_box + (uint32_t)(hch & 31) * 2 + htap;
          a_hi = wg_desc_sw64(aa);
          a_lo = wg_desc_sw64(aa + halo_cb * halo_box);
          hch += 16;
          const bool next_tap = hch == a.cin;
          hch = next_tap ? 0 : hch;
          htap += next_tap ? a.dil * 64 : 0;
        } else {
          a_hi = wg_desc_sw64(sa) + adv;
          a_lo = wg_desc_sw64(sa + S::A_BYTES) + adv;
        }
#pragma unroll
        for (int h = 0; h < 2; h++) {
          wgmma_ss<BN>(acc[h], a_lo + h * HALF, w_hi + adv, (kb | ks) != 0);
          wgmma_ss<BN>(acc[h], a_hi + h * HALF, w_lo + adv, 1);
          wgmma_ss<BN>(acc[h], a_hi + h * HALF, w_hi + adv, 1);
        }
      }
      wg_commit();
      wg_wait<1>();
      wg_fence_acc(acc[0]);
      wg_fence_acc(acc[1]);
      if (kb > 0 && et == 0) mbar_arrive(&empty[stage == 0 ? NSTAGE - 1 : stage - 1]);
      if (++stage == NSTAGE) {
        stage = 0;
        phase ^= 1;
      }
    }
    named_arrive(turn_other, 256);
    wg_wait<0>();
    wg_fence_acc(acc[0]);
    wg_fence_acc(acc[1]);
    if (et == 0) mbar_arrive(&empty[stage == 0 ? NSTAGE - 1 : stage - 1]);
    if (HALO && et == 0) mbar_arrive(&halo_empty[c]);
    const int mt = tile / a.n_tiles, nt = tile - mt * a.n_tiles;
    const bool stage_params = a.n_tiles > 1 || n == 0;
    if constexpr (POOLING) {
      tc_pool_epilogue_tile<BN, EPI>(a, params, chunk, pool_stage, acc, bar, mt, nt * BN, quad, lane, et, stage_params);
    } else if constexpr (EPI == TC_CONV2D) {
      float* acc_s = reinterpret_cast<float*>(tile_s);
      named_sync(acc_free, 256);
#pragma unroll
      for (int h = 0; h < 2; h++) {
        const int r0 = 64 * h + 16 * quad + (lane >> 2);
#pragma unroll
        for (int j = 0; j < BN / 8; j++) {
          const int col = 8 * j + 2 * (lane & 3);
          *reinterpret_cast<float2*>(acc_s + r0 * S::ACC_LD + col) = make_float2(acc[h][4 * j], acc[h][4 * j + 1]);
          *reinterpret_cast<float2*>(acc_s + (r0 + 8) * S::ACC_LD + col) = make_float2(acc[h][4 * j + 2], acc[h][4 * j + 3]);
        }
      }
      named_sync(bar, 128);
      if (stage_params) tc_stage_params<BN, EPI>(a, params, bar, nt * BN, et);
      tc_conv2d_epilogue_tile<BN>(a, params, acc_s + et * S::ACC_LD, mt, nt * BN, quad, lane);
      named_arrive(acc_free_other, 256);
    } else {
      named_sync(acc_free, 256);
      tc_box_epilogue<BN, EPI>(a, params, acc, smem_u32(tile_s), quad, lane);
      fence_proxy_async_smem();
      named_sync(bar, 128);
      if (et == 0) {
        const int m0 = mt * TC_BM, n0 = nt * BN;
        if (EPI == TC_LEAKY_BN_SPLIT) {
#pragma unroll
          for (int b = 0; b < BN / 64; b++) {
            if (n0 + 64 * b >= a.N) break;
            tma_store_2d(&tmC0, tile_s + b * S::BOX_BYTES, n0 + 64 * b, m0);
            tma_store_2d(&tmC1, tile_s + (BN / 64 + b) * S::BOX_BYTES, n0 + 64 * b, m0);
          }
        } else {
#pragma unroll
          for (int b = 0; b < BN / 32; b++) {
            if (n0 + 32 * b >= a.N) break;
            tma_store_2d(&tmC0, tile_s + b * S::BOX_BYTES, n0 + 32 * b, m0);
          }
        }
        bulk_commit();
        bulk_wait_read_all();
      }
      __syncwarp();
      named_arrive(acc_free_other, 256);
    }
  }
  if (tc_box_store(EPI) && et == 0) bulk_wait_all();
}

constexpr int TCW_N = 112;
struct TcWsSmem {
  static constexpr int W_BOX = 64 * TC_BK * 2;
  static constexpr int BAR_BYTES = 128;
  static constexpr int CHUNK_FLOATS = TCW_N * 33;
  static constexpr int STAGE_FLOATS = 64 + 2 * CHUNK_FLOATS;
  __host__ static int halo_rows(int KW, int dil) { return (TCW_N + (KW - 1) * dil + 7) / 8 * 8; }
  __host__ static int w_plane_bytes(int K) { return (K + TC_BK - 1) / TC_BK * W_BOX; }
  __host__ static int op_bytes(int cin, int KW, int dil) {
    return 2 * w_plane_bytes(KW * cin) + 2 * TcSmem<64>::halo_bytes(cin, halo_rows(KW, dil));
  }
  __host__ static int total(int op) { return op + BAR_BYTES + STAGE_FLOATS * 4 + 1024; }
};

__global__ void __launch_bounds__(TC_THREADS, 1)
gemm_tc_ws_kernel(const __grid_constant__ CUtensorMap tmA_hi, const __grid_constant__ CUtensorMap tmA_lo,
                  const __grid_constant__ CUtensorMap tmW_hi, const __grid_constant__ CUtensorMap tmW_lo, TcArgs a) {
  using S = TcWsSmem;
  extern __shared__ unsigned char smem_raw[];
  unsigned char* smem = reinterpret_cast<unsigned char*>((reinterpret_cast<uintptr_t>(smem_raw) + 1023) & ~uintptr_t(1023));
  const int w_plane = a.wblocks * S::W_BOX;
  unsigned char* halo = smem + 2 * w_plane;
  uint64_t* bars = reinterpret_cast<uint64_t*>(smem + a.op_bytes);
  uint64_t* w_full = bars;
  uint64_t* tile_full = bars + 1;
  uint64_t* tile_empty = bars + 3;
  uint64_t* halo_full = bars + 5;
  uint64_t* halo_empty = bars + 7;
  volatile int* tile_idx = reinterpret_cast<volatile int*>(bars + 9);
  float* bias_s = reinterpret_cast<float*>(reinterpret_cast<unsigned char*>(bars) + S::BAR_BYTES);

  const int warp = __shfl_sync(0xffffffffu, (int)(threadIdx.x >> 5), 0), lane = threadIdx.x & 31;
  const int wg = warp >> 2;
  const int num_tiles = a.m_tiles;
  const int halo_box = a.halo_rows * 64, halo_cb = (a.cin + 31) / 32;

  if (threadIdx.x == 0) {
    mbar_init(w_full, 1);
    for (int c = 0; c < 2; c++) {
      mbar_init(&tile_full[c], 1);
      mbar_init(&tile_empty[c], 128);
      mbar_init(&halo_full[c], 1);
      mbar_init(&halo_empty[c], 1);
    }
    asm volatile("fence.mbarrier_init.release.cluster;" ::: "memory");
  }
  if (threadIdx.x < 64) bias_s[threadIdx.x] = (int)threadIdx.x < a.N && a.bias ? a.bias[threadIdx.x] : 0.f;
  __syncthreads();

  if (wg == 0) {
    setmaxnreg_dec<40>();
    if (threadIdx.x == 0) {
      mbar_expect_tx(w_full, 2 * w_plane);
      for (int b = 0; b < a.wblocks; b++) {
        tma_load_2d(smem + b * S::W_BOX, &tmW_hi, b * TC_BK, 0, w_full);
        tma_load_2d(smem + w_plane + b * S::W_BOX, &tmW_lo, b * TC_BK, 0, w_full);
      }
      for (int i = 0, tile = blockIdx.x;; i++) {
        const int c = i & 1;
        if (tile < num_tiles) {
          mbar_wait(&halo_empty[c], ((i >> 1) & 1) ^ 1);
          unsigned char* hs = halo + c * a.halo_bytes;
          const int r0 = tile * a.tile_rows;
          mbar_expect_tx(&halo_full[c], 2 * halo_cb * halo_box);
          for (int cb = 0; cb < halo_cb; cb++) {
            tma_load_2d(hs + cb * halo_box, &tmA_hi, cb * TC_BK, r0, &halo_full[c]);
            tma_load_2d(hs + (halo_cb + cb) * halo_box, &tmA_lo, cb * TC_BK, r0, &halo_full[c]);
          }
        }
        mbar_wait(&tile_empty[c], ((i >> 1) & 1) ^ 1);
        if (tile >= num_tiles) {
          tile_idx[c] = -1;
          mbar_arrive(&tile_full[c]);
          mbar_wait(&tile_empty[c ^ 1], (((i + 1) >> 1) & 1) ^ 1);
          tile_idx[c ^ 1] = -2;
          mbar_arrive(&tile_full[c ^ 1]);
          break;
        }
        tile_idx[c] = tile;
        mbar_arrive(&tile_full[c]);
        tile = (int)gridDim.x + (int)atomicAdd(&a.tile_ctr[0], 1u);
      }
      __threadfence();
      if (atomicAdd(&a.tile_ctr[1], 1u) == gridDim.x - 1) {
        atomicExch(&a.tile_ctr[0], 0u);
        atomicExch(&a.tile_ctr[1], 0u);
      }
    }
    return;
  }
  setmaxnreg_inc<232>();
  const int c = wg - 1, quad = warp & 3, et = threadIdx.x - 128 * wg;
  const int bar = 1 + c, turn = 3 + c, turn_other = 3 + (c ^ 1);
  float* chunk = bias_s + 64 + c * S::CHUNK_FLOATS;
  if (c == 1) named_arrive(3, 256);
  const int ksteps = a.KW * a.cin / 16;
  const uint32_t w_s = smem_u32(smem), hs = smem_u32(halo + c * a.halo_bytes);
  mbar_wait(w_full, 0);
  for (int n = 0;; n++) {
    mbar_wait(&tile_full[c], n & 1);
    const int tile = tile_idx[c];
    mbar_arrive(&tile_empty[c]);
    named_sync(turn, 256);
    if (tile < 0) {
      if (tile == -1) named_arrive(turn_other, 256);
      break;
    }
    float acc[TCW_N / 2];
#pragma unroll
    for (int i = 0; i < TCW_N / 2; i++) acc[i] = 0.f;
    mbar_wait(&halo_full[c], n & 1);
    uint32_t htap = 0;
    int hch = 0;
    wg_fence_acc(acc);
    wg_fence();
    for (int s = 0; s < ksteps; s++) {
      const uint32_t wa = w_s + (uint32_t)(s >> 1) * S::W_BOX + (uint32_t)(s & 1) * 32;
      const uint64_t w_hi = wg_desc_sw64(wa), w_lo = wg_desc_sw64(wa + w_plane);
      const uint32_t xa = hs + (uint32_t)(hch >> 5) * halo_box + (uint32_t)(hch & 31) * 2 + htap;
      const uint64_t x_hi = wg_desc_sw64(xa), x_lo = wg_desc_sw64(xa + halo_cb * halo_box);
      hch += 16;
      const bool next_tap = hch == a.cin;
      hch = next_tap ? 0 : hch;
      htap += next_tap ? a.dil * 64 : 0;
      wgmma_ss<TCW_N>(acc, w_hi, x_lo, s != 0);
      wgmma_ss<TCW_N>(acc, w_lo, x_hi, 1);
      wgmma_ss<TCW_N>(acc, w_hi, x_hi, 1);
    }
    wg_commit();
    named_arrive(turn_other, 256);
    wg_wait<0>();
    wg_fence_acc(acc);
    if (et == 0) mbar_arrive(&halo_empty[c]);
    const uint32_t frag = smem_u32(chunk) + 4 * (2 * (lane & 3) * 33 + 16 * (quad & 1) + (lane >> 2));
#pragma unroll
    for (int c0 = 0; c0 < 64; c0 += 32) {
      if ((quad >> 1) == (c0 >> 5)) {
#pragma unroll
        for (int j = 0; j < TCW_N / 8; j++)
#pragma unroll
          for (int e = 0; e < 4; e++)
            st_shared_u32(frag + 4 * ((8 * j + (e & 1)) * 33 + 8 * (e >> 1)), __float_as_uint(acc[4 * j + e] * a.acc_scale));
      }
      named_sync(bar, 128);
      tc_maxpool3_cols<true>(a, chunk, chunk, bias_s + c0, tile, c0, et, bar);
    }
  }
}

static int make_map(CUtensorMap* m, const void* base, long long rows, int cols, int ld, int box_cols, int box_rows,
                    bool f32 = false) {
  EncodeTiledFn fn = encode_fn();
  if (!fn) {
    set_error("cuTensorMapEncodeTiled is not available from the driver");
    return -2;
  }
  const int esize = f32 ? 4 : 2;
  cuuint64_t dims[2] = {(cuuint64_t)cols, (cuuint64_t)rows};
  cuuint64_t strides[1] = {(cuuint64_t)ld * esize};
  cuuint32_t box[2] = {(cuuint32_t)box_cols, (cuuint32_t)box_rows};
  cuuint32_t estr[2] = {1, 1};
  CUresult r = fn(m, f32 ? CU_TENSOR_MAP_DATA_TYPE_FLOAT32 : CU_TENSOR_MAP_DATA_TYPE_BFLOAT16, 2, const_cast<void*>(base), dims,
                  strides, box, estr, CU_TENSOR_MAP_INTERLEAVE_NONE,
                  box_cols * esize == 128 ? CU_TENSOR_MAP_SWIZZLE_128B : CU_TENSOR_MAP_SWIZZLE_64B,
                  CU_TENSOR_MAP_L2_PROMOTION_L2_256B, CU_TENSOR_MAP_FLOAT_OOB_FILL_NONE);
  if (r != CUDA_SUCCESS) {
    set_error("cuTensorMapEncodeTiled failed with code " + std::to_string((int)r));
    return -2;
  }
  return 0;
}

constexpr int TC_CTR_SLOTS = 1024;
__device__ unsigned g_tc_tile_ctr[TC_CTR_SLOTS][2];

static unsigned* tile_counter(cudaStream_t st) {
  static std::mutex mu;
  static std::map<std::pair<int, cudaStream_t>, int> slot_of;
  static int used[64] = {};
  int dev = 0;
  if (cudaGetDevice(&dev) != cudaSuccess || dev < 0 || dev >= 64) {
    set_error("gemm_tc: no current CUDA device");
    return nullptr;
  }
  int slot;
  {
    std::lock_guard<std::mutex> lock(mu);
    auto it = slot_of.find({dev, st});
    if (it != slot_of.end()) {
      slot = it->second;
    } else {
      if (used[dev] == TC_CTR_SLOTS) {
        set_error("gemm_tc: more than " + std::to_string(TC_CTR_SLOTS) + " streams have launched GEMMs on one device");
        return nullptr;
      }
      slot = slot_of[{dev, st}] = used[dev]++;
    }
  }
  void* base = nullptr;
  if (cudaGetSymbolAddress(&base, g_tc_tile_ctr) != cudaSuccess) {
    set_error("gemm_tc: cannot address the tile counters");
    return nullptr;
  }
  return static_cast<unsigned*>(base) + 2 * slot;
}

static int tc_bn(const TcGemm& g) { return g.epi == TC_MAXPOOL3 || (g.Npad == 64 && g.epi == TC_BIAS_F32) ? 64 : 128; }
static int tc_halo_rows(const TcGemm& g) {
  return (TC_BM + (g.KW - ((g.KW * g.Cin) % 32 ? 0 : 1)) * g.dil + 7) / 8 * 8;
}
template <int BN>
static int tc_halo_smem(const TcGemm& g) { return TcSmem<BN>::total(g.epi, TcSmem<BN>::halo_op_bytes(g.Cin, tc_halo_rows(g))); }

bool gemm_tc_ws(const TcGemm& g) {
  if (g.epi != TC_MAXPOOL3 || g.tap_boxes || g.tap_off || g.KW < 2 || g.dil < 1 || g.Cin % 16 || g.Cin > 128 ||
      g.pool3_tile_rows > TCW_N || TcWsSmem::halo_rows(g.KW, g.dil) > 256)
    return false;
  return TcWsSmem::total(TcWsSmem::op_bytes(g.Cin, g.KW, g.dil)) <= TC_SMEM_MAX;
}

bool gemm_tc_halo(const TcGemm& g) {
  if (g.tap_boxes || g.epi == TC_CONV2D || g.tap_off || g.KW < 2 || g.dil < 1 || g.Cin % 16 || g.Cin > 128 ||
      tc_halo_rows(g) > 256)
    return false;
  return gemm_tc_ws(g) || (tc_bn(g) == 64 ? tc_halo_smem<64>(g) : tc_halo_smem<128>(g)) <= TC_SMEM_MAX;
}

static int tc_setup(const TcGemm& g, int bn, int epi, bool halo, CUtensorMap* maps, TcArgs& a, bool ws = false) {
  const int Ktot = g.KW * g.Cin, bk = TC_BK, a_rows = ws ? TcWsSmem::halo_rows(g.KW, g.dil) : (halo ? tc_halo_rows(g) : TC_BM);
  if (make_map(&maps[0], g.A_hi, g.Mtot, g.Cin, g.lda, bk, a_rows) || make_map(&maps[1], g.A_lo, g.Mtot, g.Cin, g.lda, bk, a_rows) ||
      make_map(&maps[2], g.W_hi, g.Npad, Ktot, Ktot, bk, bn) || make_map(&maps[3], g.W_lo, g.Npad, Ktot, Ktot, bk, bn))
    return -2;
  memset(&maps[4], 0, 2 * sizeof(CUtensorMap));
  if (epi == TC_LEAKY_BN_SPLIT) {
    if (make_map(&maps[4], g.out_hi, g.M, g.N, g.ldc, 64, TC_BM) || make_map(&maps[5], g.out_lo, g.M, g.N, g.ldc, 64, TC_BM))
      return -2;
  } else if (tc_box_store(epi)) {
    if (make_map(&maps[4], g.out_f32, g.M, g.N, g.ldc, 32, TC_BM, true)) return -2;
  }
  a = TcArgs{};
  a.M = g.M; a.N = g.N; a.n_tiles = (g.N + bn - 1) / bn;
  a.tile_rows = epi == TC_MAXPOOL3 ? g.pool3_tile_rows : TC_BM;
  a.pool3_T = g.pool3_T;
  a.m_tiles = (int)((g.M + a.tile_rows - 1) / a.tile_rows);
  a.KW = g.KW; a.dil = g.dil; a.cin_blocks = g.Cin / bk;
  a.bias = g.bias; a.bn_scale = g.bn_scale; a.bn_shift = g.bn_shift;
  a.out_f32 = g.out_f32; a.out_hi = reinterpret_cast<__nv_bfloat16*>(g.out_hi);
  a.out_lo = reinterpret_cast<__nv_bfloat16*>(g.out_lo); a.ldc = g.ldc;
  a.acc_scale = g.w_scale > 0.f ? 1.f / g.w_scale : 1.f;
  for (int j = 0; j < 9; j++) a.tap_off[j] = j < g.KW ? (g.tap_off ? g.tap_off[j] : j * g.dil) : 0;
  a.Wp = g.Wp; a.Hp = g.Hp; a.Wop = g.Wop; a.Hop = g.Hop; a.stride2 = g.stride2; a.relu = g.relu;
  a.res_hi = reinterpret_cast<const __nv_bfloat16*>(g.res_hi);
  a.res_lo = reinterpret_cast<const __nv_bfloat16*>(g.res_lo);
  a.pool_w = g.pool_w; a.pool_part = g.pool_part; a.pool_item_rows = g.pool_item_rows; a.pool_K = g.pool_K; a.pool_T = g.pool_T;
  a.cin = g.Cin;
  if (ws) {
    a.halo_rows = a_rows;
    a.wblocks = (Ktot + bk - 1) / bk;
    a.halo_bytes = TcSmem<64>::halo_bytes(g.Cin, a_rows);
    a.op_bytes = TcWsSmem::op_bytes(g.Cin, g.KW, g.dil);
  } else if (halo) {
    a.halo_rows = a_rows;
    a.wblocks = (Ktot + bk - 1) / bk;
    a.halo_bytes = bn == 64 ? TcSmem<64>::halo_bytes(g.Cin, a_rows) : TcSmem<128>::halo_bytes(g.Cin, a_rows);
    a.op_bytes = bn == 64 ? TcSmem<64>::halo_op_bytes(g.Cin, a_rows) : TcSmem<128>::halo_op_bytes(g.Cin, a_rows);
  } else {
    a.op_bytes = bn == 128 ? TcSmem<128>::NSTAGE * TcSmem<128>::STAGE_BYTES
                           : (bn == 64 ? TcSmem<64>::NSTAGE * TcSmem<64>::STAGE_BYTES : TcSmem<32>::NSTAGE * TcSmem<32>::STAGE_BYTES);
  }
  return 0;
}

static int tc_grid(const TcArgs& a) {
  const int sms = usable_sms();
  const int tiles = a.m_tiles * a.n_tiles;
  return tiles < sms ? tiles : sms;
}

template <int BN, int EPI, bool HALO>
static int launch_tc(const TcGemm& g, cudaStream_t st) {
  using S = TcSmem<BN>;
  CUtensorMap m[6];
  TcArgs a;
  if (tc_setup(g, BN, EPI, HALO, m, a)) return -2;
  if (tc_pooling(EPI) && !(a.tile_ctr = tile_counter(st))) return -2;
  auto kern = gemm_tc_kernel<BN, EPI, HALO>;
  static bool attr_done[64] = {};
  if (first_use_on_device(attr_done))
    DG_CUDA(cudaFuncSetAttribute(kern, cudaFuncAttributeMaxDynamicSharedMemorySize, HALO ? TC_SMEM_MAX : S::total(EPI)));
  kern<<<tc_grid(a), TC_THREADS, S::total(EPI, a.op_bytes), st>>>(m[0], m[1], m[2], m[3], m[4], m[5], a);
  DG_LAUNCHED();
  return 0;
}

static int launch_tc_ws(const TcGemm& g, cudaStream_t st) {
  CUtensorMap m[6];
  TcArgs a;
  if (tc_setup(g, 64, TC_MAXPOOL3, true, m, a, true) || !(a.tile_ctr = tile_counter(st))) return -2;
  static bool attr_done[64] = {};
  if (first_use_on_device(attr_done))
    DG_CUDA(cudaFuncSetAttribute(gemm_tc_ws_kernel, cudaFuncAttributeMaxDynamicSharedMemorySize, TC_SMEM_MAX));
  gemm_tc_ws_kernel<<<tc_grid(a), TC_THREADS, TcWsSmem::total(a.op_bytes), st>>>(m[0], m[1], m[2], m[3], a);
  DG_LAUNCHED();
  return 0;
}

template <int BN, int EPI>
static int launch_tc(const TcGemm& g, cudaStream_t st) {
  return gemm_tc_halo(g) ? launch_tc<BN, EPI, true>(g, st) : launch_tc<BN, EPI, false>(g, st);
}

int launch_gemm_tc(const TcGemm& g, cudaStream_t st) {
  ProfScope _ps(g.tag ? g.tag : "gemm_tc", st);
  if (g.Cin % (gemm_tc_halo(g) ? 16 : 64) || g.lda % 8 || g.ldc % (g.epi == TC_LEAKY_BN_SPLIT ? 8 : 4) ||
      (g.Npad % 128 && g.Npad != 64 && g.Npad != 32) || g.KW < 1 || g.KW > 9) {
    set_error("gemm_tc: Cin must be a multiple of 64 (a Conv1d of 2..9 taps over at most 128 channels whose tile halo fits "
              "in shared memory, e.g. Cin 80: a multiple of 16), A pitch a multiple of 8, output pitch a multiple of 4 "
              "(8 for 16-bit planes), padded N 32, 64 or a multiple of 128, at most 9 taps");
    return -1;
  }
  if (g.epi == TC_LEAKY_BN_SPLIT && g.N % 32) {
    set_error("gemm_tc (planes): N must be a multiple of 32");
    return -1;
  }
  if (tc_box_store(g.epi)) {
    const bool planes = g.epi == TC_LEAKY_BN_SPLIT;
    const uintptr_t base = planes ? ((uintptr_t)g.out_hi | (uintptr_t)g.out_lo) : (uintptr_t)g.out_f32;
    if (!base || (planes && (!g.out_hi || !g.out_lo)) || base % 16 || g.ldc < g.N || g.M >= (1LL << 31)) {
      set_error("gemm_tc: the output needs a 16-byte aligned base, a pitch of at least N and fewer than 2^31 rows");
      return -1;
    }
  }
  if (g.epi == TC_CONV2D) {
    if (g.ldc % 32 || g.N % 32 || g.Wp < 3 || g.Hp < 3 || (!g.out_hi && !g.out_f32) || g.M >= (1LL << 31)) {
      set_error("gemm_tc (conv2d): channel counts must be multiples of 32");
      return -1;
    }
    if (g.Npad == 32) return launch_tc<32, TC_CONV2D, false>(g, st);
    if (g.Npad == 64) return launch_tc<64, TC_CONV2D, false>(g, st);
    return launch_tc<128, TC_CONV2D, false>(g, st);
  }
  if (g.epi == TC_POOL) {
    if (g.Npad % 128 || !g.pool_w || !g.pool_part || g.pool_K < 1 || g.pool_K > 4 || g.pool_item_rows < TC_BM || g.pool_T < 1 ||
        g.pool_T > g.pool_item_rows) {
      set_error("gemm_tc (pool): needs 128-wide tiles, 1..4 speakers, items of at least 128 rows and 1..item rows valid frames");
      return -1;
    }
    return launch_tc<128, TC_POOL>(g, st);
  }
  if (g.epi == TC_MAXPOOL3) {
    if (g.Npad != 64 || !g.out_f32 || !g.pool_part || g.pool3_T < 1 || g.pool3_tile_rows < 3 || g.pool3_tile_rows > 126 ||
        g.pool3_tile_rows % 3 || g.pool_item_rows % g.pool3_tile_rows || g.M % g.pool_item_rows) {
      set_error("gemm_tc (maxpool3): needs 64 output channels and tiles of 3..126 rows (a multiple of 3) that divide the item");
      return -1;
    }
    if (gemm_tc_ws(g)) return launch_tc_ws(g, st);
    return launch_tc<64, TC_MAXPOOL3>(g, st);
  }
  if (g.Npad == 64 && g.epi == TC_BIAS_F32) return launch_tc<64, TC_BIAS_F32>(g, st);
  switch (g.epi) {
    case TC_BIAS_F32:
      return launch_tc<128, TC_BIAS_F32>(g, st);
    case TC_LEAKY_BN_SPLIT:
      return launch_tc<128, TC_LEAKY_BN_SPLIT>(g, st);
    default:
      return launch_tc<128, TC_LEAKY_BN_F32>(g, st);
  }
}

__global__ void __launch_bounds__(128) wgmma_row_shift_kernel(const __grid_constant__ CUtensorMap tmA,
                                                              const __grid_constant__ CUtensorMap tmW, int base_offset_mode,
                                                              float* out) {
  __shared__ __align__(1024) unsigned char sm[72 * 64 + 8 * 64];
  __shared__ uint64_t bar;
  if (threadIdx.x == 0) {
    mbar_init(&bar, 1);
    asm volatile("fence.mbarrier_init.release.cluster;" ::: "memory");
  }
  __syncthreads();
  if (threadIdx.x == 0) {
    mbar_expect_tx(&bar, sizeof(sm));
    tma_load_2d(sm, &tmA, 0, 0, &bar);
    tma_load_2d(sm + 72 * 64, &tmW, 0, 0, &bar);
  }
  mbar_wait(&bar, 0);
  const int w = threadIdx.x >> 5, l = threadIdx.x & 31;
  for (int r = 0; r <= 8; r++) {
    for (int ks = 0; ks < 2; ks++) {
      const uint32_t sa = smem_u32(sm) + r * 64 + ks * 32;
      uint64_t da = wg_desc_sw64(sa);
      if (base_offset_mode) da |= (uint64_t)((sa >> 7) & 7) << 49;
      const uint64_t dw = wg_desc_sw64(smem_u32(sm + 72 * 64) + ks * 32);
      float d[4] = {0.f, 0.f, 0.f, 0.f};
      wg_fence_acc(d);
      wg_fence();
      wgmma_ss<8>(d, da, dw, 0);
      wg_commit();
      wg_wait<0>();
      wg_fence_acc(d);
      for (int i = 0; i < 4; i++)
        out[((r * 2 + ks) * 64 + 16 * w + l / 4 + 8 * ((i / 2) % 2)) * 8 + 2 * (l % 4) + i % 2] = d[i];
    }
  }
}

int selftest_wgmma_row_shift(int base_offset_mode, unsigned* ok_shifts) {
  std::vector<uint16_t> A(72 * 32), W(8 * 32);
  std::vector<float> Af(A.size()), Wf(W.size());
  for (size_t i = 0; i < A.size(); i++) Af[i] = (float)((int)((i * 7 + i / 32 * 3) % 9) - 4);
  for (size_t i = 0; i < W.size(); i++) Wf[i] = (float)((int)((i * 5 + 1) % 7) - 3);
  for (size_t i = 0; i < A.size(); i++) A[i] = host_f32_to_h16(Af[i]);
  for (size_t i = 0; i < W.size(); i++) W[i] = host_f32_to_h16(Wf[i]);
  void *dA = nullptr, *dW = nullptr, *dO = nullptr;
  const size_t out_n = 9 * 2 * 64 * 8;
  int rc = 0;
  CUtensorMap mA, mW;
  if (cudaMalloc(&dA, A.size() * 2) != cudaSuccess || cudaMalloc(&dW, W.size() * 2) != cudaSuccess ||
      cudaMalloc(&dO, out_n * 4) != cudaSuccess ||
      cudaMemcpy(dA, A.data(), A.size() * 2, cudaMemcpyHostToDevice) != cudaSuccess ||
      cudaMemcpy(dW, W.data(), W.size() * 2, cudaMemcpyHostToDevice) != cudaSuccess) {
    set_error("selftest_wgmma_row_shift: device buffers");
    rc = -2;
  }
  if (!rc && (make_map(&mA, dA, 72, 32, 32, 32, 72) || make_map(&mW, dW, 8, 32, 32, 32, 8))) rc = -2;
  std::vector<float> out(out_n);
  if (!rc) {
    wgmma_row_shift_kernel<<<1, 128>>>(mA, mW, base_offset_mode, static_cast<float*>(dO));
    if (cudaDeviceSynchronize() != cudaSuccess || cudaMemcpy(out.data(), dO, out_n * 4, cudaMemcpyDeviceToHost) != cudaSuccess) {
      set_error(std::string("selftest_wgmma_row_shift: ") + cudaGetErrorString(cudaGetLastError()));
      rc = -2;
    }
  }
  cudaFree(dA);
  cudaFree(dW);
  cudaFree(dO);
  if (rc) return rc;
  *ok_shifts = 0;
  for (int r = 0; r <= 8; r++) {
    bool ok = true;
    for (int ks = 0; ks < 2; ks++)
      for (int m = 0; m < 64; m++)
        for (int n = 0; n < 8; n++) {
          float ref = 0.f;
          for (int k = 0; k < 16; k++) ref += Af[(r + m) * 32 + 16 * ks + k] * Wf[n * 32 + 16 * ks + k];
          if (out[((r * 2 + ks) * 64 + m) * 8 + n] != ref) ok = false;
        }
    if (ok) *ok_shifts |= 1u << r;
  }
  return 0;
}

__global__ void __launch_bounds__(128) wgmma_b_row_shift_kernel(const __grid_constant__ CUtensorMap tmA,
                                                                const __grid_constant__ CUtensorMap tmB, int base_offset_mode,
                                                                float* out) {
  __shared__ __align__(1024) unsigned char sm[64 * 64 + 72 * 64];
  __shared__ uint64_t bar;
  if (threadIdx.x == 0) {
    mbar_init(&bar, 1);
    asm volatile("fence.mbarrier_init.release.cluster;" ::: "memory");
  }
  __syncthreads();
  if (threadIdx.x == 0) {
    mbar_expect_tx(&bar, sizeof(sm));
    tma_load_2d(sm, &tmA, 0, 0, &bar);
    tma_load_2d(sm + 64 * 64, &tmB, 0, 0, &bar);
  }
  mbar_wait(&bar, 0);
  const int w = threadIdx.x >> 5, l = threadIdx.x & 31;
  for (int r = 0; r <= 8; r++) {
    for (int ks = 0; ks < 2; ks++) {
      const uint32_t sb = smem_u32(sm + 64 * 64) + r * 64 + ks * 32;
      uint64_t db = wg_desc_sw64(sb);
      if (base_offset_mode) db |= (uint64_t)((sb >> 7) & 7) << 49;
      const uint64_t da = wg_desc_sw64(smem_u32(sm) + ks * 32);
      float d[32];
      for (int i = 0; i < 32; i++) d[i] = 0.f;
      wg_fence_acc(d);
      wg_fence();
      wgmma_ss<64>(d, da, db, 0);
      wg_commit();
      wg_wait<0>();
      wg_fence_acc(d);
      for (int i = 0; i < 32; i++)
        out[((r * 2 + ks) * 64 + 16 * w + l / 4 + 8 * ((i / 2) % 2)) * 64 + 8 * (i / 4) + 2 * (l % 4) + i % 2] = d[i];
    }
  }
}

int selftest_wgmma_b_row_shift(int base_offset_mode, unsigned* ok_shifts) {
  std::vector<uint16_t> A(64 * 32), B(72 * 32);
  std::vector<float> Af(A.size()), Bf(B.size());
  for (size_t i = 0; i < A.size(); i++) Af[i] = (float)((int)((i * 5 + i / 32) % 7) - 3);
  for (size_t i = 0; i < B.size(); i++) Bf[i] = (float)((int)((i * 7 + i / 32 * 3) % 9) - 4);
  for (size_t i = 0; i < A.size(); i++) A[i] = host_f32_to_h16(Af[i]);
  for (size_t i = 0; i < B.size(); i++) B[i] = host_f32_to_h16(Bf[i]);
  void *dA = nullptr, *dB = nullptr, *dO = nullptr;
  const size_t out_n = 9 * 2 * 64 * 64;
  int rc = 0;
  CUtensorMap mA, mB;
  if (cudaMalloc(&dA, A.size() * 2) != cudaSuccess || cudaMalloc(&dB, B.size() * 2) != cudaSuccess ||
      cudaMalloc(&dO, out_n * 4) != cudaSuccess ||
      cudaMemcpy(dA, A.data(), A.size() * 2, cudaMemcpyHostToDevice) != cudaSuccess ||
      cudaMemcpy(dB, B.data(), B.size() * 2, cudaMemcpyHostToDevice) != cudaSuccess) {
    set_error("selftest_wgmma_b_row_shift: device buffers");
    rc = -2;
  }
  if (!rc && (make_map(&mA, dA, 64, 32, 32, 32, 64) || make_map(&mB, dB, 72, 32, 32, 32, 72))) rc = -2;
  std::vector<float> out(out_n);
  if (!rc) {
    wgmma_b_row_shift_kernel<<<1, 128>>>(mA, mB, base_offset_mode, static_cast<float*>(dO));
    if (cudaDeviceSynchronize() != cudaSuccess || cudaMemcpy(out.data(), dO, out_n * 4, cudaMemcpyDeviceToHost) != cudaSuccess) {
      set_error(std::string("selftest_wgmma_b_row_shift: ") + cudaGetErrorString(cudaGetLastError()));
      rc = -2;
    }
  }
  cudaFree(dA);
  cudaFree(dB);
  cudaFree(dO);
  if (rc) return rc;
  *ok_shifts = 0;
  for (int r = 0; r <= 8; r++) {
    bool ok = true;
    for (int ks = 0; ks < 2; ks++)
      for (int m = 0; m < 64; m++)
        for (int n = 0; n < 64; n++) {
          float ref = 0.f;
          for (int k = 0; k < 16; k++) ref += Af[m * 32 + 16 * ks + k] * Bf[(r + n) * 32 + 16 * ks + k];
          if (out[((r * 2 + ks) * 64 + m) * 64 + n] != ref) ok = false;
        }
    if (ok) *ok_shifts |= 1u << r;
  }
  return 0;
}

__global__ void __launch_bounds__(256) split_kernel(const float* __restrict__ x, long long rows_out, int C, int ld_in,
                                                    int ld_out, int pool, int item_rows, const float* __restrict__ sc,
                                                    const float* __restrict__ sh, __nv_bfloat16* __restrict__ hi,
                                                    __nv_bfloat16* __restrict__ lo, const int* __restrict__ skip_flag) {
  if (skip_flag && *skip_flag != 0) return;
  const int q_per_row = ld_out >> 2;
  const long long n4 = rows_out * q_per_row;
  for (long long i = (long long)blockIdx.x * blockDim.x + threadIdx.x; i < n4; i += (long long)gridDim.x * blockDim.x) {
    const long long row = i / q_per_row;
    const int c = (int)(i - row * q_per_row) << 2;
    float4 v = make_float4(0.f, 0.f, 0.f, 0.f);
    if (c < C) {
      if (pool) {
        const float* p = x + (row * 3) * ld_in + c;
        const float4 a = *reinterpret_cast<const float4*>(p), b = *reinterpret_cast<const float4*>(p + ld_in),
                     d = *reinterpret_cast<const float4*>(p + 2 * ld_in);
        v = make_float4(fmaxf(fmaxf(a.x, b.x), d.x), fmaxf(fmaxf(a.y, b.y), d.y), fmaxf(fmaxf(a.z, b.z), d.z),
                        fmaxf(fmaxf(a.w, b.w), d.w));
      } else {
        v = *reinterpret_cast<const float4*>(x + row * ld_in + c);
      }
      if (sc) {
        const long long item = row / item_rows;
        const float4 s = *reinterpret_cast<const float4*>(sc + item * ld_in + c);
        const float4 h = *reinterpret_cast<const float4*>(sh + item * ld_in + c);
        v.x = leaky(fmaf(v.x, s.x, h.x)); v.y = leaky(fmaf(v.y, s.y, h.y));
        v.z = leaky(fmaf(v.z, s.z, h.z)); v.w = leaky(fmaf(v.w, s.w, h.w));
      }
    }
    uint16_t h0, h1, h2, h3, l0, l1, l2, l3;
    split_h16(v.x, h0, l0);
    split_h16(v.y, h1, l1);
    split_h16(v.z, h2, l2);
    split_h16(v.w, h3, l3);
    reinterpret_cast<uint2*>(hi)[i] = make_uint2(pack_u16x2(h0, h1), pack_u16x2(h2, h3));
    reinterpret_cast<uint2*>(lo)[i] = make_uint2(pack_u16x2(l0, l1), pack_u16x2(l2, l3));
  }
}

int launch_split_ex(const float* x, long long rows_out, int C, int ld_in, int ld_out, int pool, int item_rows,
                    const float* sc, const float* sh, void* hi, void* lo, cudaStream_t st, const int* skip_flag) {
  ProfScope _ps("split16", st);
  if (C % 4 || ld_in % 4 || ld_out % 4) {
    set_error("split: channel counts must be multiples of 4");
    return -1;
  }
  const long long n4 = rows_out * (ld_out / 4);
  const long long want = (n4 + 255) / 256;
  const int cap = usable_sms() * 16;
  const int grid = (int)(want < cap ? want : cap);
  split_kernel<<<grid, 256, 0, st>>>(x, rows_out, C, ld_in, ld_out, pool, item_rows, sc, sh,
                                     reinterpret_cast<__nv_bfloat16*>(hi), reinterpret_cast<__nv_bfloat16*>(lo), skip_flag);
  DG_LAUNCHED();
  return 0;
}

uint16_t host_f32_to_h16(float f) {
  uint32_t u;
  memcpy(&u, &f, 4);
  const uint32_t sign = (u >> 16) & 0x8000u;
  const uint32_t au = u & 0x7FFFFFFFu;
  if (au > 0x7F800000u) return (uint16_t)(sign | 0x7FFFu);
  if (au >= 0x477FF000u) return (uint16_t)(sign | 0x7BFFu);
  if (au < 0x33000001u) return (uint16_t)sign;
  const int e = (int)(au >> 23) - 127;
  uint32_t mant = (au & 0x7FFFFFu) | 0x800000u;
  int shift = e >= -14 ? 13 : 13 + (-14 - e);
  uint32_t q = mant >> shift;
  const uint32_t rem = mant & ((1u << shift) - 1u), half = 1u << (shift - 1);
  if (rem > half || (rem == half && (q & 1u))) q++;
  const uint32_t bits = e >= -14 ? (uint32_t)((e + 14) << 10) + q : q;
  return (uint16_t)(sign | bits);
}
float host_h16_to_f32(uint16_t h) {
  const uint32_t sign = ((uint32_t)h & 0x8000u) << 16, e = (h >> 10) & 31u, m = h & 0x3FFu;
  if (e == 0) {
    const float v = (float)m * 5.9604644775390625e-08f;
    return sign ? -v : v;
  }
  const uint32_t u = e == 31 ? (sign | 0x7F800000u | (m << 13)) : (sign | ((e + 112u) << 23) | (m << 13));
  float f;
  memcpy(&f, &u, 4);
  return f;
}

void split_weights_host(const float* w, int N, int Npad, int K, uint16_t* hi, uint16_t* lo, float scale) {
  for (size_t i = 0; i < (size_t)Npad * K; i++) hi[i] = lo[i] = 0;
  for (int n = 0; n < N; n++)
    for (int k = 0; k < K; k++) {
      const float f = w[(size_t)n * K + k] * scale;
      const uint16_t h = host_f32_to_h16(f);
      hi[(size_t)n * K + k] = h;
      lo[(size_t)n * K + k] = host_f32_to_h16(f - host_h16_to_f32(h));
    }
}

float weight_plane_scale(const float* w, size_t n) {
  float mx = 0.f;
  for (size_t i = 0; i < n; i++) {
    const float v = fabsf(w[i]);
    if (v > mx && v < 3.0e38f) mx = v;
  }
  if (!(mx > 0.f)) return 1.f;
  int e = 0;
  frexpf(mx, &e);
  int k = 13 - e;
  k = k > 40 ? 40 : (k < -40 ? -40 : k);
  return ldexpf(1.f, k);
}

}
```

### include/diart_b200.h

```cpp
#ifndef DIART_B200_H
#define DIART_B200_H

#include <stddef.h>
#include <stdint.h>

#ifdef __cplusplus
extern "C" {
#endif

#define DG_OK 0
#define DG_EINVAL (-1)
#define DG_ECUDA (-2)
#define DG_EWEIGHT (-3)
#define DG_ENCCL (-4)

typedef struct dg_tensor {
  const char* name;
  const float* data;
  int64_t numel;
} dg_tensor;

typedef struct dg_seg dg_seg;
typedef struct dg_emb dg_emb;
typedef struct dg_cluster dg_cluster;
typedef struct dg_pipeline dg_pipeline;
typedef struct dg_post dg_post;
typedef struct dg_stream dg_stream;
typedef struct dg_sweep dg_sweep;
typedef struct dg_vad_sweep dg_vad_sweep;

const char* dg_last_error(void);
int dg_version(void);

int dg_seg_create(const dg_tensor* tensors, int n_tensors, int device, dg_seg** out);
int dg_seg_dims(const dg_seg* h, int num_samples, int* frames, int* speakers);
int dg_seg_set_powerset(dg_seg* h, int num_speakers, int max_per_frame);
int dg_seg_forward(dg_seg* h, const float* wav_dev , int B, int S,
                   float* seg_dev , void* stream);
int dg_seg_destroy(dg_seg* h);

int dg_emb_create(const dg_tensor* tensors, int n_tensors, int pool_mode, int device, dg_emb** out);
int dg_emb_dims(const dg_emb* h, int num_samples, int* frames, int* dimension);
int dg_emb_forward(dg_emb* h, const float* wav_dev , const float* weights_dev, int B, int S,
                   int F, int K, int normalize, float norm, float* out_dev, void* stream);
int dg_emb_forward_rows(dg_emb* h, const float* wav_dev , const float* weights_dev ,
                        int N, int S, int F, float* out_dev , void* stream);
int dg_emb_destroy(dg_emb* h);
int dg_emb_debug_trunk(dg_emb* h, const float* wav_dev, int U, int S, int stop_after, float* out_host, int64_t cap, int* dims);
int dg_seg_debug_stage(dg_seg* h, const float* wav_dev, int B, int S, int hop, int stage, float* out_host, int64_t cap, int* dims);
int dg_emb_debug_stage(dg_emb* h, const float* wav_dev, const float* weights_dev, int B, int S, int F, int K, int hop, int stage,
                       float* out_host, int64_t cap, int* dims);

int dg_osp(const float* seg_dev , int B, int F, int K, float gamma, float beta,
           int normalize, float* out_dev, void* stream);
int dg_normalize_embeddings(const float* emb_dev , int rows, int D, float norm,
                            float* out_dev, void* stream);

int dg_cluster_create(int max_speakers, int dim, double tau_active, double rho_update,
                      double delta_new, int device, dg_cluster** out);
int dg_cluster_set_metric(dg_cluster* h, int metric);
int dg_cluster_step(dg_cluster* h, const float* seg_dev , const float* emb_dev ,
                    int B, int F, int K, int32_t* map_dev, float* permuted_dev, void* stream);
int dg_cluster_reset(dg_cluster* h);
int dg_cluster_get_state(dg_cluster* h, double* centers_host, int32_t* active_host, int* initialized);
int dg_cluster_set_state(dg_cluster* h, const double* centers_host, const int32_t* active_host, int initialized);
int dg_cluster_destroy(dg_cluster* h);

int dg_pipeline_create(dg_seg* seg, dg_emb* emb, dg_cluster* clu, float gamma, float beta,
                       int normalize_weights, dg_pipeline** out);
int dg_pipeline_step(dg_pipeline* h, const float* wav_dev , int B, int S,
                     float* seg_dev , float* emb_dev ,
                     int32_t* map_dev , float* permuted_dev , void* stream);
int dg_pipeline_set_hop(dg_pipeline* h, int hop_samples);
int dg_pipeline_step_host(dg_pipeline* h, const float* wav_host, int B, int S, float* seg_host,
                          float* emb_host, int32_t* map_host, float* permuted_host );
int dg_pipeline_submit(dg_pipeline* h, const float* wav_dev , int B, int S,
                       void* stream);
int dg_pipeline_collect(dg_pipeline* h, const float** seg_dev, const float** emb_dev, const int32_t** map_dev,
                        void* stream);
int dg_pipeline_collect_copy(dg_pipeline* h, float* seg_dev, float* emb_dev, int32_t* map_dev, void* stream);
int dg_pipeline_submit_host(dg_pipeline* h, const float* wav_host , int B, int S);
int dg_pipeline_collect_host(dg_pipeline* h, float* seg_host, float* emb_host, int32_t* map_host);
int dg_pipeline_nets_sets(dg_pipeline* h, const float* wav_dev, int B, int S, int num_sets, const float* osp_host,
                          const int32_t* normalize_host, float* seg_dev, float* emb_dev, int64_t emb_set_stride, void* stream);
int dg_pipeline_destroy(dg_pipeline* h);

int dg_post_create(int frames, int local_speakers, int max_speakers, int num_windows, const double* hamming_host,
                   double tau, int device, dg_post** out);
int dg_post_step(dg_post* h, const float* seg_dev , const int32_t* map_dev , int B,
                 const int32_t* plan_host, int32_t* header_host, uint32_t* turns_host, int turn_cap_host, int* n_turns,
                 void* stream);
int dg_post_reset(dg_post* h);
int dg_post_destroy(dg_post* h);
int dg_pipeline_call_host(dg_pipeline* h, dg_post* post, const float* const* rows_host, int B, int S,
                          const int32_t* plan_host, int32_t* header_host, uint32_t* turns_host, int turn_cap_host,
                          int* n_turns, float* seg_host , int32_t* map_host );
int64_t dg_pipeline_last_call_h2d_bytes(const dg_pipeline* h);

int dg_sweep_create(int max_speakers, int dim, int frames, int local_speakers, int num_windows, const double* hamming_host,
                    int device, dg_sweep** out);
int dg_sweep_run(dg_sweep* h, const float* seg_dev, const float* emb_dev, int N, const double* params_host, int T,
                 const int32_t* plan_host, int32_t* maps_dev, double* centers_dev, int32_t* header_host, uint32_t* turns_host,
                 int turn_cap_host, int* n_turns, void* stream);
int dg_sweep_destroy(dg_sweep* h);
int dg_sweep_set_scored_regions(dg_sweep* h, int num_files, const double* rows_host, const int32_t* offsets_host);
int dg_vad_sweep_set_scored_regions(dg_vad_sweep* h, int num_files, const double* rows_host, const int32_t* offsets_host);
int dg_sweep_set_trial_sets(dg_sweep* h, int num_sets, const int32_t* trial_set_host, int T);
int dg_sweep_set_seeds(dg_sweep* h, int num_files, const int32_t* offsets_host, const double* centers_host);
int dg_sweep_set_identities(dg_sweep* h, int num_files, const int32_t* hyp_of_ref_host);
int dg_sweep_score(dg_sweep* h, const float* seg_dev, const float* emb_dev, int N, const double* params_host, int T,
                   const int32_t* plan_host, const double* out_start_host, const double* out_res_host, double shift,
                   double collar, const double* ref_host, const int32_t* ref_label_host, int S, int R,
                   double* components_host, int32_t* hyp_offsets_dev, double* hyp_segments_dev, int hyp_cap, void* stream);
int dg_sweep_run_files(dg_sweep* h, const float* seg_dev, const float* emb_dev, int N, int num_files,
                       const int32_t* chunk_offsets_host, const double* params_host, int T, const int32_t* plan_host,
                       int32_t* maps_dev, double* centers_dev, int32_t* header_host, uint32_t* turns_host, int turn_cap_host,
                       int* n_turns, void* stream);
int dg_sweep_score_files(dg_sweep* h, const float* seg_dev, const float* emb_dev, int N, int num_files,
                         const int32_t* chunk_offsets_host, const double* params_host, int T, const int32_t* plan_host,
                         const double* out_start_host, const double* out_res_host, const double* shifts_host, double collar,
                         const double* ref_host, const int32_t* ref_label_host, const int32_t* ref_offsets_host,
                         const int32_t* ref_label_counts_host, double* components_host, int32_t* hyp_offsets_dev,
                         double* hyp_segments_dev, int hyp_cap, void* stream);
int dg_sweep_state_order(int num_files, const int32_t* chunk_offsets_host, int T, int32_t* states_host);
int dg_sweep_run_latencies(dg_sweep* h, const float* seg_dev, const float* emb_dev, int N, int num_units,
                           const int32_t* unit_offsets_host, int num_virtual, int num_virtual_files, const int32_t* vchunk_host,
                           const int32_t* virtual_offsets_host, const double* params_host, int T, const int32_t* plan_host,
                           int32_t* maps_dev, int32_t* header_host, uint32_t* turns_host, int turn_cap_host, int* n_turns,
                           void* stream);
int dg_sweep_score_latencies(dg_sweep* h, const float* seg_dev, const float* emb_dev, int N, int num_units,
                             const int32_t* unit_offsets_host, int num_virtual, int num_virtual_files,
                             const int32_t* vchunk_host, const int32_t* virtual_offsets_host, const double* params_host, int T,
                             const int32_t* plan_host, const double* out_start_host, const double* out_res_host,
                             const double* shifts_host, double collar, const double* ref_host, const int32_t* ref_label_host,
                             const int32_t* ref_offsets_host, const int32_t* ref_label_counts_host, double* components_host,
                             void* stream);
int dg_sweep_check_latencies(int N, int num_units, const int32_t* unit_offsets_host, int num_virtual, int num_virtual_files,
                             const int32_t* vchunk_host, const int32_t* virtual_offsets_host, const int32_t* plan_host,
                             int num_windows, int frames);
int dg_vad_sweep_create(int frames, int local_speakers, int num_windows, const double* hamming_host, int device,
                        dg_vad_sweep** out);
int dg_vad_sweep_curve(dg_vad_sweep* h, const float* seg_dev, int N, int num_files, const int32_t* chunk_offsets_host,
                       const int32_t* plan_host, void* stream);
int dg_vad_sweep_curve_latencies(dg_vad_sweep* h, const float* seg_dev, int N, int num_units, const int32_t* unit_offsets_host,
                                 int num_virtual, int num_virtual_files, const int32_t* vchunk_host,
                                 const int32_t* virtual_offsets_host, const int32_t* plan_host, void* stream);
int dg_vad_sweep_run_files(dg_vad_sweep* h, const double* taus_host, int T, int32_t* header_host, uint32_t* turns_host,
                           int turn_cap_host, int* n_turns, void* stream);
int dg_vad_sweep_score_files(dg_vad_sweep* h, const double* taus_host, int T, const double* out_start_host,
                             const double* out_res_host, const double* shifts_host, double collar, const double* ref_host,
                             const int32_t* ref_offsets_host, double* components_host, void* stream);
int dg_vad_sweep_destroy(dg_vad_sweep* h);

int dg_stream_create(int chunk_samples, int step_samples, int max_windows, int device, dg_stream** out);
int dg_stream_push_host(dg_stream* h, const float* samples_host, int n);
int dg_stream_available(const dg_stream* h);
int dg_stream_windows(dg_stream* h, int B, float* wav_dev, void* stream);
int dg_stream_reset(dg_stream* h);
int dg_stream_destroy(dg_stream* h);
int dg_pipeline_submit_stream(dg_pipeline* h, dg_stream* stream, int B);
int dg_pipeline_call_stream(dg_pipeline* h, dg_post* post, dg_stream* stream, int B, const int32_t* plan_host,
                            int32_t* header_host, uint32_t* turns_host, int turn_cap_host, int* n_turns,
                            float* seg_host , int32_t* map_host );

typedef struct dg_multi dg_multi;
int dg_multi_create(dg_seg* seg, dg_emb* emb, int chunk_samples, int step_samples, int max_streams, int max_windows_per_stream,
                    int max_speakers, double tau, double rho, double delta, float gamma, float beta, int normalize_weights,
                    int num_windows, const double* hamming_host, dg_multi** out);
int dg_multi_open(dg_multi* h, int slot);
int dg_multi_close(dg_multi* h, int slot);
int dg_multi_push_host(dg_multi* h, int slot, const float* samples_host, int n);
int dg_multi_available(const dg_multi* h, int slot);
int dg_multi_step(dg_multi* h, const int32_t* plan_host, int n_rows, int32_t* counts_host, int32_t* header_host,
                  uint32_t* turns_host, int turn_cap_host, int* n_turns, float* seg_dev ,
                  float* emb_dev , int32_t* map_dev );
int dg_multi_last_step_ms(const dg_multi* h, float* ms);
int dg_multi_destroy(dg_multi* h);
typedef struct dg_resample dg_resample;
int dg_multi_add_rate(dg_multi* h, dg_resample* rs, int chunk_samples, int step_samples, int* rate_id);
int dg_multi_open_rate(dg_multi* h, int slot, int rate_id);
int dg_multi_open_config(dg_multi* h, int slot, int rate_id, int num_windows, const double params[3] );
int dg_multi_open_seeded(dg_multi* h, int slot, int rate_id, int num_windows, const double params[3] ,
                         const double* centers_host , int n);
int dg_multi_get_state(dg_multi* h, int slot, double* centers_host , int32_t* active_host ,
                       int* initialized);
typedef struct dg_gallery dg_gallery;
int dg_gallery_create(const double* centroids_host, int G, int D, int device, dg_gallery** out);
int dg_gallery_destroy(dg_gallery* g);
int dg_gallery_query(dg_gallery* g, const double* queries_dev , int Q, const int32_t* group_dev ,
                     const int32_t* claimed_dev , double threshold, int32_t* entry_dev ,
                     double* dist_dev , void* stream);
int dg_multi_set_gallery(dg_multi* h, dg_gallery* g, double threshold);
int dg_multi_set_slot_gallery(dg_multi* h, int slot, dg_gallery* g, double threshold);
int dg_multi_set_names(dg_multi* h, int slot, uint32_t named, const int32_t* claimed_host );
int dg_multi_last_names(const dg_multi* h, int32_t* out_host , int cap, int* n);
int dg_multi_last_windows(const dg_multi* h, float* wav_dev, int n_rows);
int dg_multi_export_bytes(const dg_multi* h, const int32_t* slots, int n, int64_t* bytes_out);
int dg_multi_export(dg_multi* h, const int32_t* slots, int n, int close, void* out_host, int64_t out_bytes);
int dg_multi_import(dg_multi* h, const void* blob_host, int64_t blob_bytes, int n, dg_gallery* const* gals,
                    int32_t* slots_out);
int dg_selftest_multi_transfer_host(const int32_t* geom, int n_ops, const int32_t* ops, const float* samples_host,
                                    int32_t* result, int src_slot, int patch, float* ring_out, float* yring_out, float* hist_out,
                                    int64_t cap, int64_t* info, char* message, int msg_cap);
int dg_selftest_multi_frames_host(int slots, int max_wps, int out_chunk, int out_step, int n_rates, const int32_t* rates,
                                  int n_ops, const int32_t* ops, int32_t* result, int64_t* records, int cap, int* n_records);
int dg_selftest_multi_staging_host(int slots, int C, int n_ops, const int32_t* ops, const float* samples_host, int32_t* result,
                                   float* rings_host);
int dg_selftest_gallery_plan_host(int n, const int32_t* slots, int n_keys, const int32_t* G, const double* thr,
                                  int32_t* groups_out, int32_t* segs_out, int32_t* work_out, int cap, int32_t* counts);
int dg_selftest_multi_gallery_host(int slots, int D, int M, int n_gal, const int32_t* gal, int n_ops, const double* ops,
                                   int32_t* result, char* messages, int msg_cap);
int dg_multi_create_vad(dg_seg* seg, int chunk_samples, int step_samples, int max_streams, int max_windows_per_stream,
                        double tau, int num_windows, const double* hamming_host, dg_multi** out);

typedef struct dg_resample dg_resample;
int dg_resample_create(int orig_rate, int new_rate, const float* taps_host, int width, int device, dg_resample** out);
int64_t dg_resample_out_len(const dg_resample* h, int64_t num_samples);
int dg_resample_forward(dg_resample* h, const float* in_dev, int B, int64_t L, float* out_dev, void* stream);
int dg_resample_destroy(dg_resample* h);
int dg_stream_create_resampled(int chunk_samples, int step_samples, dg_resample* rs, int max_windows, int device,
                               dg_stream** out);
int dg_stream_crop_host(dg_stream* h, int n, const int64_t* ranges_host, float* out_host);

int64_t dg_launch_count(void);
int dg_profile_enable(int enable);
int dg_selftest_gemm_tc(int M, int Cin, int KW, int dil, int N, int epi, float* max_abs_diff, float* out_rms);
int dg_selftest_gemm_tc_grid(int M, int Cin, int KW, int dil, int N, int epi, int* equal);
int dg_selftest_gemm_tc_bounds(int M, int Cin, int N, int epi, int* outside_unchanged, int* equal, int* refused);
int dg_selftest_wgmma_row_shift(int base_offset_mode, unsigned* ok_shifts);
int dg_selftest_wgmma_b_row_shift(int base_offset_mode, unsigned* ok_shifts);
int dg_selftest_gemm_tc_halo(int M, int Cin, int KW, int dil, int N, int epi, int* equal, int* halo);
int dg_selftest_gemm_tc_pool3_simt(int M, int Cin, int KW, int dil, int N, float* max_abs_diff, float* out_rms, int* ws);
int dg_selftest_split_f16_host(const float* x, long long n, unsigned short* hi, unsigned short* lo);
int dg_selftest_sinc_filters_host(const float* low_hz, const float* band_hz, float* filters);
int dg_selftest_fbank_tables_host(float* frame_operator, float* mel_banks);
int dg_profile_report(char* buf, int cap);

int dg_cluster_record_len(const dg_cluster* h);
int dg_cluster_export_delta(dg_cluster* h, double* record_dev, void* stream);
int dg_cluster_merge(dg_cluster* h, const double* records_dev , int world, int rank,
                     int32_t* maps_dev , int n_maps, void* stream);
int dg_pipeline_identity_export(dg_pipeline* h, double* record_dev, void* stream);
int dg_pipeline_identity_merge(dg_pipeline* h, const double* records_dev, int world, int rank, void* stream);

#ifdef __cplusplus
}
#endif
#endif
```

Measured before the change: 23340.

## Add resident-weight mode for 1x1 tensor-core GEMMs with per-column tile scheduling

Adds a new kernel variant for KW=1 box-store GEMMs. Each CTA is pinned to one 128-column slice, loads that slice's full weight panel into shared memory once, and then streams only A tiles through a deeper ring. Row tiles are handed out through per-column atomic counters, and the epilogue is done in two 64-column halves so it fits the smaller staging tile. The aim is to stop reloading weight tiles for every M tile and to save TMA bandwidth. The cost is more shared memory, a grid fixed to a multiple of n_tiles that may leave SMs idle, and extra counter reset logic. A selftest for the new mode is also added.

New measurement: 23730, median of 6. 1.02x the previous value.

```diff
diff --git a/diart_b200/_lib.py b/diart_b200/_lib.py
--- a/diart_b200/_lib.py
+++ b/diart_b200/_lib.py
@@ -35,6 +35,8 @@
                                                  C.POINTER(C.c_float), C.POINTER(C.c_int)]),
     "dg_selftest_gemm_tc_halo": (C.c_int, [C.c_int, C.c_int, C.c_int, C.c_int, C.c_int, C.c_int, C.POINTER(C.c_int),
                                            C.POINTER(C.c_int)]),
+    "dg_selftest_gemm_tc_resident": (C.c_int, [C.c_int, C.c_int, C.c_int, C.c_int, C.c_int, C.c_int, C.c_int,
+                                               C.POINTER(C.c_int), C.POINTER(C.c_int)]),
     "dg_selftest_split_f16_host": (C.c_int, [_P, C.c_longlong, _P, _P]),
     "dg_seg_create": (C.c_int, [C.POINTER(DgTensor), C.c_int, C.c_int, C.POINTER(_P)]),
     "dg_seg_dims": (C.c_int, [_P, C.c_int, C.POINTER(C.c_int), C.POINTER(C.c_int)]),
diff --git a/diart_b200/csrc/api.cu b/diart_b200/csrc/api.cu
--- a/diart_b200/csrc/api.cu
+++ b/diart_b200/csrc/api.cu
@@ -458,6 +458,68 @@
     else if (cur != first)
       *equal = 0;
   }
+  return DG_OK;
+}
+
+extern "C" int dg_selftest_gemm_tc_resident(int M, int Cin, int KW, int dil, int N, int epi, int sm_cap, int* equal,
+                                            int* resident) {
+  if (M < 1 || Cin < 64 || Cin % 64 || KW < 1 || KW > 9 || dil < 1 || N < 1 || N % 4 || epi < 0 || epi > 2 ||
+      (epi == 1 && N % 32) || sm_cap < 0 || !equal || !resident) {
+    set_error("dg_selftest_gemm_tc_resident: bad arguments");
+    return DG_EINVAL;
+  }
+  const int K = KW * Cin, npad = N <= 64 && epi == 0 ? 64 : (N + 127) / 128 * 128;
+  uint32_t seed = 31337u;
+  auto rnd = [&]() {
+    seed = seed * 1664525u + 1013904223u;
+    return ((seed >> 8) & 0xFFFF) / 65536.f - 0.5f;
+  };
+  std::vector<float> A((size_t)M * Cin), Wnk((size_t)N * K), bias(N), bsc(N), bsh(N);
+  for (auto& v : A) v = 2.f * rnd();
+  for (auto& v : Wnk) v = 0.25f * rnd();
+  for (int n = 0; n < N; n++) {
+    bias[n] = rnd();
+    bsc[n] = 1.f + rnd();
+    bsh[n] = rnd();
+  }
+  const size_t f32_bytes = epi == 1 ? 0 : (size_t)M * N * 4, plane_bytes = epi == 1 ? (size_t)M * N * 2 : 0;
+  DevBuf dA, dAh, dAl, dB, dS, dH, dF, dOh, dOl;
+  WeightPlanes dW;
+  if (upload(dA, A) || upload(dB, bias) || upload(dS, bsc) || upload(dH, bsh) || upload_split(dW, Wnk, N, npad, K))
+    return DG_ECUDA;
+  if (dAh.ensure((size_t)M * Cin * 2) || dAl.ensure((size_t)M * Cin * 2) || dF.ensure(f32_bytes + 4) ||
+      dOh.ensure(plane_bytes + 4) || dOl.ensure(plane_bytes + 4))
+    return DG_ECUDA;
+  int rc;
+  if ((rc = launch_split_ex(dA.as<float>(), M, Cin, Cin, Cin, 0, 1, nullptr, nullptr, dAh.p, dAl.p, nullptr))) return rc;
+  TcGemm t{};
+  t.A_hi = dAh.p; t.A_lo = dAl.p; t.lda = Cin; t.Cin = Cin; t.KW = KW; t.dil = dil; t.Mtot = M; t.M = M;
+  t.N = N; t.bias = dB.as<float>(); t.bn_scale = dS.as<float>(); t.bn_shift = dH.as<float>(); t.ldc = N;
+  t.epi = epi; t.tag = "selftest_tc_resident";
+  t.out_f32 = f32_bytes ? dF.as<float>() : nullptr;
+  t.out_hi = plane_bytes ? dOh.p : nullptr;
+  t.out_lo = plane_bytes ? dOl.p : nullptr;
+  if ((rc = set_weights(t, dW))) return rc;
+  *resident = gemm_tc_resident(t) ? 1 : 0;
+  TcGemm ref = t;
+  ref.tap_boxes = 1;
+  std::vector<unsigned char> first, cur;
+  for (int run = 0; run < 2; run++) {
+    DG_CUDA(cudaMemset(dF.p, 0, f32_bytes + 4));
+    DG_CUDA(cudaMemset(dOh.p, 0, plane_bytes + 4));
+    DG_CUDA(cudaMemset(dOl.p, 0, plane_bytes + 4));
+    {
+      SmLimit cap(run == 0 ? sm_cap : 0);
+      if ((rc = launch_gemm_tc(run == 0 ? t : ref, nullptr))) return rc;
+    }
+    DG_CUDA(cudaDeviceSynchronize());
+    cur.resize(f32_bytes + 2 * plane_bytes);
+    DG_CUDA(cudaMemcpy(cur.data(), dF.p, f32_bytes, cudaMemcpyDeviceToHost));
+    DG_CUDA(cudaMemcpy(cur.data() + f32_bytes, dOh.p, plane_bytes, cudaMemcpyDeviceToHost));
+    DG_CUDA(cudaMemcpy(cur.data() + f32_bytes + plane_bytes, dOl.p, plane_bytes, cudaMemcpyDeviceToHost));
+    if (run == 0) first.swap(cur);
+  }
+  *equal = cur == first ? 1 : 0;
   return DG_OK;
 }
 
diff --git a/diart_b200/csrc/dg_common.cuh b/diart_b200/csrc/dg_common.cuh
--- a/diart_b200/csrc/dg_common.cuh
+++ b/diart_b200/csrc/dg_common.cuh
@@ -149,6 +149,7 @@
 int launch_gemm_tc(const TcGemm& g, cudaStream_t st);
 bool gemm_tc_halo(const TcGemm& g);
 bool gemm_tc_ws(const TcGemm& g);
+bool gemm_tc_resident(const TcGemm& g);
 int selftest_wgmma_row_shift(int base_offset_mode, unsigned* ok_shifts);
 int selftest_wgmma_b_row_shift(int base_offset_mode, unsigned* ok_shifts);
 int launch_split_ex(const float* x, long long rows_out, int C, int ld_in, int ld_out, int pool, int item_rows,
diff --git a/diart_b200/csrc/gemm_tc.cu b/diart_b200/csrc/gemm_tc.cu
--- a/diart_b200/csrc/gemm_tc.cu
+++ b/diart_b200/csrc/gemm_tc.cu
@@ -53,6 +53,8 @@
 __host__ __device__ constexpr bool tc_pooling(int epi) { return epi == TC_POOL || epi == TC_MAXPOOL3; }
 __host__ __device__ constexpr bool tc_box_store(int epi) { return epi == TC_BIAS_F32 || epi == TC_LEAKY_BN_SPLIT || epi == TC_LEAKY_BN_F32; }
 
+enum TcOps { TC_OPS_TAPS = 0, TC_OPS_HALO = 1, TC_OPS_RESIDENT = 2 };
+
 template <int BN>
 struct TcSmem {
   static constexpr int A_BYTES = TC_BM * TC_BK * 2;
@@ -83,27 +85,48 @@
               TcSmem<32>::total(TC_CONV2D) <= TC_SMEM_MAX && TcSmem<128>::total(TC_BIAS_F32) <= TC_SMEM_MAX,
               "gemm_tc: shared memory");
 
+struct TcResSmem {
+  using S = TcSmem<128>;
+  static constexpr int MIN_STAGES = 4, MAX_STAGES = 10;
+  static constexpr int STAGE_BYTES = 2 * S::A_BYTES;
+  static constexpr int HALF_COLS = 64;
+  static constexpr int STAGE_TILE_BYTES = TC_BM * HALF_COLS * 4;
+  static constexpr int FIXED_BYTES = STAGE_TILE_BYTES + S::BAR_BYTES + S::PARAM_FLOATS * 4 + 1024;
+  __host__ __device__ static constexpr int stages(int kblocks) {
+    return (TC_SMEM_MAX - FIXED_BYTES - kblocks * S::W_STAGE_BYTES) / STAGE_BYTES < MAX_STAGES
+               ? (TC_SMEM_MAX - FIXED_BYTES - kblocks * S::W_STAGE_BYTES) / STAGE_BYTES
+               : MAX_STAGES;
+  }
+  __host__ __device__ static constexpr int op_bytes(int kblocks) { return kblocks * S::W_STAGE_BYTES + stages(kblocks) * STAGE_BYTES; }
+  __host__ __device__ static constexpr int total(int kblocks) { return op_bytes(kblocks) + FIXED_BYTES; }
+};
+static_assert(TcResSmem::stages(256 / TC_BK) >= TcResSmem::MIN_STAGES && TcResSmem::total(256 / TC_BK) <= TC_SMEM_MAX &&
+              2 * TcResSmem::MAX_STAGES * 8 + 6 * 8 + 8 <= TcSmem<128>::BAR_BYTES, "gemm_tc: resident-W shared memory");
+
+template <int BN, int EPI>
+__device__ __forceinline__ void tc_stage_param(const TcArgs& a, float* params, int n0, int i) {
+  const int n = n0 + i;
+  const bool ok = n < a.N;
+  params[i] = (ok && a.bias) ? a.bias[n] : 0.f;
+  constexpr bool has_bn = EPI != TC_BIAS_F32;
+  params[BN + i] = (ok && has_bn) ? a.bn_scale[n] * (EPI == TC_CONV2D ? a.acc_scale : 1.f) : 1.f;
+  params[2 * BN + i] = (ok && has_bn) ? a.bn_shift[n] : 0.f;
+}
 template <int BN, int EPI>
 __device__ __forceinline__ void tc_stage_params(const TcArgs& a, float* params, int bar, int n0, int et) {
   named_sync(bar, 128);
-  for (int i = et; i < BN; i += 128) {
-    const int n = n0 + i;
-    const bool ok = n < a.N;
-    params[i] = (ok && a.bias) ? a.bias[n] : 0.f;
-    constexpr bool has_bn = EPI != TC_BIAS_F32;
-    params[BN + i] = (ok && has_bn) ? a.bn_scale[n] * (EPI == TC_CONV2D ? a.acc_scale : 1.f) : 1.f;
-    params[2 * BN + i] = (ok && has_bn) ? a.bn_shift[n] : 0.f;
-  }
+  for (int i = et; i < BN; i += 128) tc_stage_param<BN, EPI>(a, params, n0, i);
   named_sync(bar, 128);
 }
 
-template <int BN, int EPI>
+template <int BN, int EPI, int J0 = 0, int NJ = BN / 8>
 __device__ __forceinline__ void tc_box_epilogue(const TcArgs& a, const float* params, float (&acc)[2][BN / 2],
                                                 uint32_t tile, int quad, int lane) {
   using S = TcSmem<BN>;
   const int r0 = 16 * quad + (lane >> 2), sw = lane >> 2, cq = lane & 3;
 #pragma unroll
-  for (int j = 0; j < BN / 8; j++) {
+  for (int jj = 0; jj < NJ; jj++) {
+    const int j = J0 + jj;
     const int col = 8 * j + 2 * cq;
     const float2 bias = *reinterpret_cast<const float2*>(params + col);
     float2 bsc = make_float2(1.f, 1.f), bsh = make_float2(0.f, 0.f);
@@ -126,17 +149,39 @@
           uint16_t h0, l0, h1, l1;
           split_h16(x0, h0, l0);
           split_h16(x1, h1, l1);
-          const int off = (j / 8) * S::BOX_BYTES + row * 128 + (((j & 7) ^ sw) << 4) + 4 * cq;
+          const int off = (jj / 8) * S::BOX_BYTES + row * 128 + (((jj & 7) ^ sw) << 4) + 4 * cq;
           st_shared_u32(tile + off, pack_u16x2(h0, h1));
-          st_shared_u32(tile + (BN / 64) * S::BOX_BYTES + off, pack_u16x2(l0, l1));
+          st_shared_u32(tile + (NJ / 8) * S::BOX_BYTES + off, pack_u16x2(l0, l1));
         } else {
-          const int q = 2 * (j & 3) + (cq >> 1);
-          const int off = (j / 4) * S::BOX_BYTES + row * 128 + ((q ^ sw) << 4) + 8 * (cq & 1);
+          const int q = 2 * (jj & 3) + (cq >> 1);
+          const int off = (jj / 4) * S::BOX_BYTES + row * 128 + ((q ^ sw) << 4) + 8 * (cq & 1);
           st_shared_v2(tile + off, x0, x1);
         }
       }
     }
   }
+}
+
+template <int COLS, int EPI>
+__device__ __forceinline__ void tc_store_boxes(const CUtensorMap* tmC0, const CUtensorMap* tmC1, unsigned char* tile, int n0,
+                                               int m0, int N) {
+  using S = TcSmem<COLS>;
+  if (EPI == TC_LEAKY_BN_SPLIT) {
+#pragma unroll
+    for (int b = 0; b < COLS / 64; b++) {
+      if (n0 + 64 * b >= N) break;
+      tma_store_2d(tmC0, tile + b * S::BOX_BYTES, n0 + 64 * b, m0);
+      tma_store_2d(tmC1, tile + (COLS / 64 + b) * S::BOX_BYTES, n0 + 64 * b, m0);
+    }
+  } else {
+#pragma unroll
+    for (int b = 0; b < COLS / 32; b++) {
+      if (n0 + 32 * b >= N) break;
+      tma_store_2d(tmC0, tile + b * S::BOX_BYTES, n0 + 32 * b, m0);
+    }
+  }
+  bulk_commit();
+  bulk_wait_read_all();
 }
 
 __device__ __forceinline__ void acc_ld32(const float* p, uint32_t (&r)[32]) {
@@ -408,26 +453,30 @@
     }
 }
 
-template <int BN, int EPI, bool HALO>
+template <int BN, int EPI, int OPS>
 __global__ void __launch_bounds__(TC_THREADS, 1)
 gemm_tc_kernel(const __grid_constant__ CUtensorMap tmA_hi, const __grid_constant__ CUtensorMap tmA_lo,
                const __grid_constant__ CUtensorMap tmW_hi, const __grid_constant__ CUtensorMap tmW_lo,
                const __grid_constant__ CUtensorMap tmC0, const __grid_constant__ CUtensorMap tmC1, TcArgs a) {
   using S = TcSmem<BN>;
+  using R = TcResSmem;
   constexpr bool POOLING = tc_pooling(EPI);
-  constexpr int NSTAGE = HALO ? S::NSTAGE_HALO : S::NSTAGE;
+  constexpr bool HALO = OPS == TC_OPS_HALO, RESIDENT = OPS == TC_OPS_RESIDENT;
+  static_assert(!RESIDENT || (BN == 128 && tc_box_store(EPI)), "gemm_tc: the resident-W mode runs 128-column box epilogues");
+  constexpr int NSTAGE = HALO ? S::NSTAGE_HALO : (RESIDENT ? R::MAX_STAGES : S::NSTAGE);
   extern __shared__ unsigned char smem_raw[];
   unsigned char* smem = reinterpret_cast<unsigned char*>((reinterpret_cast<uintptr_t>(smem_raw) + 1023) & ~uintptr_t(1023));
-  unsigned char* ring = HALO ? smem + 2 * a.halo_bytes : smem;
-  constexpr int RING_STAGE = HALO ? S::W_STAGE_BYTES : S::STAGE_BYTES;
+  unsigned char* ring = HALO ? smem + 2 * a.halo_bytes : (RESIDENT ? smem + a.cin_blocks * S::W_STAGE_BYTES : smem);
+  constexpr int RING_STAGE = HALO ? S::W_STAGE_BYTES : (RESIDENT ? R::STAGE_BYTES : S::STAGE_BYTES);
   unsigned char* tile_s = smem + a.op_bytes;
-  uint64_t* bars = reinterpret_cast<uint64_t*>(tile_s + S::stage_tile_bytes(EPI));
+  uint64_t* bars = reinterpret_cast<uint64_t*>(tile_s + (RESIDENT ? R::STAGE_TILE_BYTES : S::stage_tile_bytes(EPI)));
   uint64_t* full = bars;
   uint64_t* empty = bars + NSTAGE;
   uint64_t* tile_full = bars + 2 * NSTAGE;
   uint64_t* tile_empty = tile_full + 2;
   uint64_t* halo_full = tile_empty + 2;
   uint64_t* halo_empty = halo_full + 2;
+  uint64_t* w_full = halo_full;
   volatile int* tile_idx = reinterpret_cast<volatile int*>(halo_empty + 2);
   float* cons = reinterpret_cast<float*>(reinterpret_cast<unsigned char*>(bars) + S::BAR_BYTES);
 
@@ -436,6 +485,7 @@
   const int num_tiles = a.m_tiles * a.n_tiles;
   const int kblocks = HALO ? a.wblocks : a.KW * a.cin_blocks;
   const int halo_box = a.halo_rows * 64, halo_cb = (a.cin + 31) / 32;
+  const int nstage = RESIDENT ? R::stages(a.cin_blocks) : NSTAGE;
 
   if (threadIdx.x == 0) {
     for (int s = 0; s < NSTAGE; s++) {
@@ -450,6 +500,7 @@
     }
     asm volatile("fence.mbarrier_init.release.cluster;" ::: "memory");
   }
+  if (RESIDENT && threadIdx.x < BN) tc_stage_param<BN, EPI>(a, cons, (int)(blockIdx.x % a.n_tiles) * BN, threadIdx.x);
   __syncthreads();
 
   if (wg == 0) {
@@ -457,6 +508,14 @@
     if (threadIdx.x == 0) {
       int stage = 0, phase = 0, next = 0;
       bool halo_next = false;
+      if constexpr (RESIDENT) {
+        const int n0 = (int)(blockIdx.x % a.n_tiles) * BN;
+        mbar_expect_tx(w_full, kblocks * S::W_STAGE_BYTES);
+        for (int kb = 0; kb < kblocks; kb++) {
+          tma_load_2d(smem + kb * S::W_STAGE_BYTES, &tmW_hi, kb * TC_BK, n0, w_full);
+          tma_load_2d(smem + kb * S::W_STAGE_BYTES + S::W_BYTES, &tmW_lo, kb * TC_BK, n0, w_full);
+        }
+      }
       for (int i = 0, tile = blockIdx.x;; i++) {
         const int c = i & 1;
         mbar_wait(&tile_empty[c], ((i >> 1) & 1) ^ 1);
@@ -509,7 +568,20 @@
             }
           }
         }
-        for (int j = 0; j < (HALO ? 0 : a.KW); j++) {
+        if constexpr (RESIDENT) {
+          for (int cb = 0; cb < a.cin_blocks; cb++) {
+            mbar_wait(&empty[stage], phase ^ 1);
+            unsigned char* st = ring + stage * RING_STAGE;
+            mbar_expect_tx(&full[stage], RING_STAGE);
+            tma_load_2d(st, &tmA_hi, cb * TC_BK, m0, &full[stage]);
+            tma_load_2d(st + S::A_BYTES, &tmA_lo, cb * TC_BK, m0, &full[stage]);
+            if (++stage == nstage) {
+              stage = 0;
+              phase ^= 1;
+            }
+          }
+        }
+        for (int j = 0; j < (HALO || RESIDENT ? 0 : a.KW); j++) {
           for (int cb = 0; cb < a.cin_blocks; cb++) {
             mbar_wait(&empty[stage], phase ^ 1);
             unsigned char* st = smem + stage * S::STAGE_BYTES;
@@ -525,7 +597,8 @@
             }
           }
         }
-        if (!HALO) next = POOLING ? (int)gridDim.x + (int)atomicAdd(&a.tile_ctr[0], 1u) : tile + (int)gridDim.x;
+        if (RESIDENT) next = ((int)gridDim.x / a.n_tiles + (int)atomicAdd(&a.tile_ctr[nt], 1u)) * a.n_tiles + nt;
+        else if (!HALO) next = POOLING ? (int)gridDim.x + (int)atomicAdd(&a.tile_ctr[0], 1u) : tile + (int)gridDim.x;
         tile = next;
       }
       if (POOLING) {
@@ -535,12 +608,17 @@
           atomicExch(&a.tile_ctr[1], 0u);
         }
       }
+      if (RESIDENT) {
+        __threadfence();
+        if (atomicAdd(&a.tile_ctr[a.n_tiles], 1u) == gridDim.x - 1)
+          for (int s = 0; s <= a.n_tiles; s++) atomicExch(&a.tile_ctr[s], 0u);
+      }
     }
     return;
   }
   setmaxnreg_inc<HALO ? 224 : 232>();
   const int c = wg - 1, quad = warp & 3, et = threadIdx.x - 128 * wg;
-  float* params = cons + c * S::consumer_floats(EPI);
+  float* params = cons + (RESIDENT ? 0 : c * S::consumer_floats(EPI));
   float* chunk = params + S::PARAM_FLOATS;
   float* pool_stage = chunk + S::CHUNK_FLOATS;
   const int bar = 1 + c, turn = 3 + c, turn_other = 3 + (c ^ 1), acc_free = 5 + c, acc_free_other = 5 + (c ^ 1);
@@ -548,11 +626,13 @@
     named_arrive(3, 256);
     if (!POOLING) named_arrive(5, 256);
   }
+  const uint32_t w_res = smem_u32(smem);
+  if (RESIDENT) mbar_wait(w_full, 0);
   for (int n = 0;; n++) {
     mbar_wait(&tile_full[c], n & 1);
     const int tile = tile_idx[c];
     mbar_arrive(&tile_empty[c]);
-    if (tc_box_store(EPI) && tile >= 0 && (a.n_tiles > 1 || n == 0))
+    if (tc_box_store(EPI) && !RESIDENT && tile >= 0 && (a.n_tiles > 1 || n == 0))
       tc_stage_params<BN, EPI>(a, params, bar, (tile - tile / a.n_tiles * a.n_tiles) * BN, et);
     named_sync(turn, 256);
     if (tile < 0) {
@@ -563,7 +643,7 @@
       break;
     }
     const int pos = (2 * n + c) * kblocks;
-    int stage = pos % NSTAGE, phase = (pos / NSTAGE) & 1;
+    int stage = pos % nstage, phase = (pos / nstage) & 1;
     float acc[2][BN / 2];
 #pragma unroll
     for (int i = 0; i < BN / 2; i++) acc[0][i] = acc[1][i] = 0.f;
@@ -574,7 +654,7 @@
     for (int kb = 0; kb < kblocks; kb++) {
       mbar_wait(&full[stage], phase);
       const uint32_t sa = smem_u32(ring + stage * RING_STAGE);
-      const uint32_t sw = HALO ? sa : sa + 2 * S::A_BYTES;
+      const uint32_t sw = RESIDENT ? w_res + kb * S::W_STAGE_BYTES : (HALO ? sa : sa + 2 * S::A_BYTES);
       const uint64_t w_hi = wg_desc_sw64(sw), w_lo = wg_desc_sw64(sw + S::W_BYTES);
       constexpr uint64_t HALF = (uint64_t)((64 * TC_BK * 2) >> 4);
       wg_fence_acc(acc[0]);
@@ -607,8 +687,8 @@
       wg_wait<1>();
       wg_fence_acc(acc[0]);
       wg_fence_acc(acc[1]);
-      if (kb > 0 && et == 0) mbar_arrive(&empty[stage == 0 ? NSTAGE - 1 : stage - 1]);
-      if (++stage == NSTAGE) {
+      if (kb > 0 && et == 0) mbar_arrive(&empty[stage == 0 ? nstage - 1 : stage - 1]);
+      if (++stage == nstage) {
         stage = 0;
         phase ^= 1;
       }
@@ -617,7 +697,7 @@
     wg_wait<0>();
     wg_fence_acc(acc[0]);
     wg_fence_acc(acc[1]);
-    if (et == 0) mbar_arrive(&empty[stage == 0 ? NSTAGE - 1 : stage - 1]);
+    if (et == 0) mbar_arrive(&empty[stage == 0 ? nstage - 1 : stage - 1]);
     if (HALO && et == 0) mbar_arrive(&halo_empty[c]);
     const int mt = tile / a.n_tiles, nt = tile - mt * a.n_tiles;
     const bool stage_params = a.n_tiles > 1 || n == 0;
@@ -640,30 +720,26 @@
       if (stage_params) tc_stage_params<BN, EPI>(a, params, bar, nt * BN, et);
       tc_conv2d_epilogue_tile<BN>(a, params, acc_s + et * S::ACC_LD, mt, nt * BN, quad, lane);
       named_arrive(acc_free_other, 256);
+    } else if constexpr (RESIDENT) {
+      constexpr int HJ = R::HALF_COLS / 8;
+      named_sync(acc_free, 256);
+      tc_box_epilogue<BN, EPI, 0, HJ>(a, params, acc, smem_u32(tile_s), quad, lane);
+      fence_proxy_async_smem();
+      named_sync(bar, 128);
+      if (et == 0) tc_store_boxes<R::HALF_COLS, EPI>(&tmC0, &tmC1, tile_s, nt * BN, mt * TC_BM, a.N);
+      named_sync(bar, 128);
+      tc_box_epilogue<BN, EPI, HJ, HJ>(a, params, acc, smem_u32(tile_s), quad, lane);
+      fence_proxy_async_smem();
+      named_sync(bar, 128);
+      if (et == 0) tc_store_boxes<R::HALF_COLS, EPI>(&tmC0, &tmC1, tile_s, nt * BN + R::HALF_COLS, mt * TC_BM, a.N);
+      __syncwarp();
+      named_arrive(acc_free_other, 256);
     } else {
       named_sync(acc_free, 256);
       tc_box_epilogue<BN, EPI>(a, params, acc, smem_u32(tile_s), quad, lane);
       fence_proxy_async_smem();
       named_sync(bar, 128);
-      if (et == 0) {
-        const int m0 = mt * TC_BM, n0 = nt * BN;
-        if (EPI == TC_LEAKY_BN_SPLIT) {
-#pragma unroll
-          for (int b = 0; b < BN / 64; b++) {
-            if (n0 + 64 * b >= a.N) break;
-            tma_store_2d(&tmC0, tile_s + b * S::BOX_BYTES, n0 + 64 * b, m0);
-            tma_store_2d(&tmC1, tile_s + (BN / 64 + b) * S::BOX_BYTES, n0 + 64 * b, m0);
-          }
-        } else {
-#pragma unroll
-          for (int b = 0; b < BN / 32; b++) {
-            if (n0 + 32 * b >= a.N) break;
-            tma_store_2d(&tmC0, tile_s + b * S::BOX_BYTES, n0 + 32 * b, m0);
-          }
-        }
-        bulk_commit();
-        bulk_wait_read_all();
-      }
+      if (et == 0) tc_store_boxes<BN, EPI>(&tmC0, &tmC1, tile_s, nt * BN, mt * TC_BM, a.N);
       __syncwarp();
       named_arrive(acc_free_other, 256);
     }
@@ -843,8 +919,8 @@
   return 0;
 }
 
-constexpr int TC_CTR_SLOTS = 1024;
-__device__ unsigned g_tc_tile_ctr[TC_CTR_SLOTS][2];
+constexpr int TC_CTR_SLOTS = 1024, TC_CTR_WORDS = 16;
+__device__ unsigned g_tc_tile_ctr[TC_CTR_SLOTS][TC_CTR_WORDS];
 
 static unsigned* tile_counter(cudaStream_t st) {
   static std::mutex mu;
@@ -874,7 +950,7 @@
     set_error("gemm_tc: cannot address the tile counters");
     return nullptr;
   }
-  return static_cast<unsigned*>(base) + 2 * slot;
+  return static_cast<unsigned*>(base) + TC_CTR_WORDS * slot;
 }
 
 static int tc_bn(const TcGemm& g) { return g.epi == TC_MAXPOOL3 || (g.Npad == 64 && g.epi == TC_BIAS_F32) ? 64 : 128; }
@@ -896,6 +972,13 @@
       tc_halo_rows(g) > 256)
     return false;
   return gemm_tc_ws(g) || (tc_bn(g) == 64 ? tc_halo_smem<64>(g) : tc_halo_smem<128>(g)) <= TC_SMEM_MAX;
+}
+
+bool gemm_tc_resident(const TcGemm& g) {
+  if (g.KW != 1 || g.tap_boxes || g.tap_off || !tc_box_store(g.epi) || tc_bn(g) != 128 || g.Cin % 64 ||
+      (g.N + 127) / 128 > TC_CTR_WORDS - 1)
+    return false;
+  return TcResSmem::stages(g.Cin / TC_BK) >= TcResSmem::MIN_STAGES && TcResSmem::total(g.Cin / TC_BK) <= TC_SMEM_MAX;
 }
 
 static int tc_setup(const TcGemm& g, int bn, int epi, bool halo, CUtensorMap* maps, TcArgs& a, bool ws = false) {
@@ -949,18 +1032,26 @@
   return tiles < sms ? tiles : sms;
 }
 
-template <int BN, int EPI, bool HALO>
+static int tc_resident_grid(const TcArgs& a) {
+  const int per_slice = std::max(1, std::min(usable_sms() / a.n_tiles, a.m_tiles));
+  return per_slice * a.n_tiles;
+}
+
+template <int BN, int EPI, int OPS>
 static int launch_tc(const TcGemm& g, cudaStream_t st) {
   using S = TcSmem<BN>;
+  constexpr bool HALO = OPS == TC_OPS_HALO, RESIDENT = OPS == TC_OPS_RESIDENT;
   CUtensorMap m[6];
   TcArgs a;
   if (tc_setup(g, BN, EPI, HALO, m, a)) return -2;
-  if (tc_pooling(EPI) && !(a.tile_ctr = tile_counter(st))) return -2;
-  auto kern = gemm_tc_kernel<BN, EPI, HALO>;
+  if ((tc_pooling(EPI) || RESIDENT) && !(a.tile_ctr = tile_counter(st))) return -2;
+  if (RESIDENT) a.op_bytes = TcResSmem::op_bytes(a.cin_blocks);
+  auto kern = gemm_tc_kernel<BN, EPI, OPS>;
   static bool attr_done[64] = {};
   if (first_use_on_device(attr_done))
-    DG_CUDA(cudaFuncSetAttribute(kern, cudaFuncAttributeMaxDynamicSharedMemorySize, HALO ? TC_SMEM_MAX : S::total(EPI)));
-  kern<<<tc_grid(a), TC_THREADS, S::total(EPI, a.op_bytes), st>>>(m[0], m[1], m[2], m[3], m[4], m[5], a);
+    DG_CUDA(cudaFuncSetAttribute(kern, cudaFuncAttributeMaxDynamicSharedMemorySize, OPS != TC_OPS_TAPS ? TC_SMEM_MAX : S::total(EPI)));
+  const int smem = RESIDENT ? TcResSmem::total(a.cin_blocks) : S::total(EPI, a.op_bytes);
+  kern<<<RESIDENT ? tc_resident_grid(a) : tc_grid(a), TC_THREADS, smem, st>>>(m[0], m[1], m[2], m[3], m[4], m[5], a);
   DG_LAUNCHED();
   return 0;
 }
@@ -979,7 +1070,10 @@
 
 template <int BN, int EPI>
 static int launch_tc(const TcGemm& g, cudaStream_t st) {
-  return gemm_tc_halo(g) ? launch_tc<BN, EPI, true>(g, st) : launch_tc<BN, EPI, false>(g, st);
+  if (gemm_tc_halo(g)) return launch_tc<BN, EPI, TC_OPS_HALO>(g, st);
+  if constexpr (BN == 128 && tc_box_store(EPI))
+    if (gemm_tc_resident(g)) return launch_tc<BN, EPI, TC_OPS_RESIDENT>(g, st);
+  return launch_tc<BN, EPI, TC_OPS_TAPS>(g, st);
 }
 
 int launch_gemm_tc(const TcGemm& g, cudaStream_t st) {
@@ -1008,9 +1102,9 @@
       set_error("gemm_tc (conv2d): channel counts must be multiples of 32");
       return -1;
     }
-    if (g.Npad == 32) return launch_tc<32, TC_CONV2D, false>(g, st);
-    if (g.Npad == 64) return launch_tc<64, TC_CONV2D, false>(g, st);
-    return launch_tc<128, TC_CONV2D, false>(g, st);
+    if (g.Npad == 32) return launch_tc<32, TC_CONV2D, TC_OPS_TAPS>(g, st);
+    if (g.Npad == 64) return launch_tc<64, TC_CONV2D, TC_OPS_TAPS>(g, st);
+    return launch_tc<128, TC_CONV2D, TC_OPS_TAPS>(g, st);
   }
   if (g.epi == TC_POOL) {
     if (g.Npad % 128 || !g.pool_w || !g.pool_part || g.pool_K < 1 || g.pool_K > 4 || g.pool_item_rows < TC_BM || g.pool_T < 1 ||
diff --git a/include/diart_b200.h b/include/diart_b200.h
--- a/include/diart_b200.h
+++ b/include/diart_b200.h
@@ -230,6 +230,7 @@
 int dg_selftest_wgmma_row_shift(int base_offset_mode, unsigned* ok_shifts);
 int dg_selftest_wgmma_b_row_shift(int base_offset_mode, unsigned* ok_shifts);
 int dg_selftest_gemm_tc_halo(int M, int Cin, int KW, int dil, int N, int epi, int* equal, int* halo);
+int dg_selftest_gemm_tc_resident(int M, int Cin, int KW, int dil, int N, int epi, int sm_cap, int* equal, int* resident);
 int dg_selftest_gemm_tc_pool3_simt(int M, int Cin, int KW, int dil, int N, float* max_abs_diff, float* out_rms, int* ws);
 int dg_selftest_split_f16_host(const float* x, long long n, unsigned short* hi, unsigned short* lo);
 int dg_selftest_sinc_filters_host(const float* low_hz, const float* band_hz, float* filters);
```
